# probabilists/zuko

Hardware: AMD Instinct MI355X
Metric: log_prob samples/sec, NSF d=64 K=8 bins=8 batch=2^20 (higher is better)
Workload: dtype f32; 1 GPU; NSF(features=64, context=0, transforms=8, bins=8, hidden=[256]*3) log_prob, batch=2^20 per GPU, x~N(0,1), seed-0 init; batch_per_gpu=1048576, global_batch=1048576, parallelism=batch-sharded x1, one RCCL all-reduce of the scalar NLL

## Files before the change

include/zuko_amd.h:

```cpp
#ifndef ZUKO_AMD_H
#define ZUKO_AMD_H

#include <stdint.h>

#ifdef __cplusplus
extern "C" {
#endif

#define ZK_DTYPE_F32 0
#define ZK_DTYPE_F64 1
#define ZK_DTYPE_BF16 2

#define ZK_ACT_NONE 0
#define ZK_ACT_RELU 1
#define ZK_ACT_ELU 2
#define ZK_ACT_TANH 3
#define ZK_ACT_SILU 4
#define ZK_ACT_GELU 5
#define ZK_ACT_SIGMOID 6
#define ZK_ACT_LEAKY 7


int zk_rqs_forward(int dtype, int64_t N, int64_t D, int K, double bound, double slope, const void* x,
                   const void* widths, int64_t w_sN, int64_t w_sD, const void* heights, int64_t h_sN, int64_t h_sD,
                   const void* derivs, int64_t d_sN, int64_t d_sD, void* y, void* ladj, int ladj_reduced,
                   int32_t* bin_out, void* stream);

int zk_rqs_inverse(int dtype, int64_t N, int64_t D, int K, double bound, double slope, const void* y,
                   const void* widths, int64_t w_sN, int64_t w_sD, const void* heights, int64_t h_sN, int64_t h_sD,
                   const void* derivs, int64_t d_sN, int64_t d_sD, void* x, int32_t* bin_out, void* stream);

int zk_rqs_from_knots(int dtype, int inverse, int64_t N, int64_t D, int K, const void* in, const void* horizontal,
                      const void* vertical, const void* slopes, int64_t k_sN, int64_t k_sD, void* out, void* ladj,
                      int32_t* bin_out, void* stream);

int zk_rqs_diag(int inverse, int64_t N, int64_t D, int K, double bound, double slope, const void* in, const void* widths,
                int64_t w_sN, int64_t w_sD, const void* heights, int64_t h_sN, int64_t h_sD, const void* derivs, int64_t d_sN,
                int64_t d_sD, void* out, void* ladj, int32_t* bin_out, float* knots_out, void* stream);

int zk_affine_forward(int dtype, int64_t N, int64_t D, double slope, const void* x, const void* shift, int64_t s_sN,
                      int64_t s_sD, const void* scale, int64_t c_sN, int64_t c_sD, void* y, void* ladj, int ladj_reduced,
                      void* stream);
int zk_affine_inverse(int dtype, int64_t N, int64_t D, double slope, const void* y, const void* shift, int64_t s_sN,
                      int64_t s_sD, const void* scale, int64_t c_sN, int64_t c_sD, void* x, void* stream);

int zk_sos_forward(int dtype, int64_t N, int64_t D, int P, int L1, double slope, const double* gl_nodes01,
                   const double* gl_weights01, const void* x, const void* a_coef, int64_t a_sN, int64_t a_sD,
                   const void* constant, int64_t c_sN, int64_t c_sD, void* y, void* ladj, int ladj_reduced, void* stream);
int zk_sos_inverse(int dtype, int64_t N, int64_t D, int P, int L1, double slope, const double* gl_nodes01,
                   const double* gl_weights01, int n_bisect, const void* y, const void* a_coef, int64_t a_sN,
                   int64_t a_sD, const void* constant, int64_t c_sN, int64_t c_sD, void* x, void* stream);

int zk_bernstein_forward(int dtype, int64_t N, int64_t D, int M, int bounded, double bound, double eps, const void* x,
                         const void* theta, int64_t t_sN, int64_t t_sD, void* y, void* ladj, int ladj_reduced, void* stream);
int zk_bernstein_inverse(int dtype, int64_t N, int64_t D, int M, int bounded, double bound, double eps, int n_bisect, const void* y,
                         const void* theta, int64_t t_sN, int64_t t_sD, void* x, void* stream);

int zk_gauss_forward(int dtype, int64_t N, int64_t D, int K, const void* x, const void* shift, int64_t b_sN, int64_t b_sD,
                     const void* scale, int64_t a_sN, int64_t a_sD, void* y, void* ladj, int ladj_reduced, void* stream);
int zk_gauss_inverse(int dtype, int64_t N, int64_t D, int K, double bound, int n_bisect, const void* y, const void* shift,
                     int64_t b_sN, int64_t b_sD, const void* scale, int64_t a_sN, int64_t a_sD, void* x, void* stream);

int zk_linear(int dtype, int64_t N, int in_features, int out_features, const void* x, int64_t ldx, const void* weight,
              const uint8_t* mask, const void* bias, int act, void* y, int64_t ldy, void* stream);

int zk_linear_bf16(int64_t N, int in_features, int out_features, const void* x, int64_t ldx, const void* weight, const uint64_t* tile_live_mask,
                   const void* bias, int act, void* y, int64_t ldy, void* stream);

int zk_linear_bf16_rqs(int64_t N, int in_features, int panels, const void* h, int64_t ldh, const void* weight_panels, const uint64_t* tile_live_mask,
                       const void* bias_panels, int K, int features, double bound, double slope, const void* x, int64_t ldx, void* y, int64_t ldy,
                       float* partial, float* ladj, void* stream);
int zk_linear_bf16_rqs_lanes(int64_t N, int in_features, int panels, const void* h, int64_t ldh, const void* weight_panels,
                             const uint64_t* tile_live_mask, const void* bias_panels, int K, int features, double bound, double slope, const void* x,
                             int64_t ldx, void* y, int64_t ldy, float* partial, float* ladj, void* stream);

typedef struct zk_ar_args_v1 {
  uint32_t struct_size;
  uint32_t version;
  int32_t uni_kind;
  int32_t D;
  int32_t DIN;
  int32_t n_layers;
  int32_t n_groups;
  int32_t n_chunks;
  int32_t act;
  int32_t bias_floats;
  int32_t accumulate;
  int32_t rev;
  int32_t n_sched;
  int32_t g0;
  int32_t g1;
  int32_t reserved;
  int64_t N;
  int64_t ldx;
  int64_t ldy;
  int64_t ldo;
  int64_t ldphi;
  double bound;
  double slope;
  const void* x;
  void* y;
  void* ladj;
  const void* y_in;
  void* x_out;
  const void* wstream;
  const void* bias;
  const uint32_t* skip;
  const int32_t* featmap;
  int32_t* bin_out;
  float* knots_out;
  const int32_t* sched;
  const int32_t* olim;
  const void* launcher;
  void* h1;
  void* h2;
  void* h3;
  void* phi;
  void* gh1;
  void* gh2;
  void* gh3;
  int32_t phi_packed;
  int32_t pad_;
  const double* gl_nodes01;
  const double* gl_weights01;
  double eps;
  double wdescale0;
  double wdescale1;
  double wdescale2;
  double wdescale3;
  uint32_t* amax0;
  uint32_t* amax1;
  uint32_t* amax2;
  uint32_t* amax3;
  const void* base_loc;
  const void* base_scale;
} zk_ar_args_v1;

int zk_ar_forward(const zk_ar_args_v1* args, void* stream);
int zk_ar_forward_split(const zk_ar_args_v1* args, void* stream);
int zk_ar_forward_diag(const zk_ar_args_v1* args, void* stream);
int zk_ar_dgrad_chain(const zk_ar_args_v1* args, void* stream);
int zk_ar_dgrad_full(const zk_ar_args_v1* args, void* stream);
int zk_ar_backward_full(const zk_ar_args_v1* args, void* stream);
int zk_ar_inverse_sweep(const zk_ar_args_v1* args, void* stream);
int zk_ar_inverse_partial(const zk_ar_args_v1* args, void* stream);
typedef struct zk_coupling_args_v1 {
  uint32_t struct_size;
  uint32_t version;
  int32_t D;
  int32_t C;
  int32_t nit;
  int32_t n_groups;
  int32_t n_layers;
  int32_t n_chunks;
  int32_t act;
  int32_t bias_floats;
  int32_t accumulate;
  int32_t static_ok;
  int64_t N;
  int64_t ldx;
  int64_t ldc;
  int64_t ldy;
  double slope;
  const void* in;
  const void* ctx;
  void* out;
  void* ladj;
  const void* wstream;
  const void* bias;
  const int32_t* bias_off;
  const int32_t* amap;
  const int32_t* fmap;
  const int32_t* tiles;
  const int32_t* widths;
  double wdescale0;
  double wdescale1;
  double wdescale2;
  double wdescale3;
} zk_coupling_args_v1;
int zk_coupling_forward(const zk_coupling_args_v1* args, void* stream);
int zk_coupling_inverse(const zk_coupling_args_v1* args, void* stream);
typedef struct zk_ar_inc_args_v1 {
  uint32_t struct_size;
  uint32_t version;
  int32_t uni_kind;
  int32_t n_hidden;
  int32_t D;
  int32_t C;
  int32_t n_groups;
  int32_t n_chunks;
  int32_t act;
  int32_t bias_floats;
  int64_t N;
  int64_t ldy;
  int64_t ldc;
  int64_t ldx;
  double bound;
  double slope;
  const void* y;
  const void* ctx;
  void* x;
  void* ladj;
  const void* wstream;
  const void* bias;
  const int32_t* bias_off;
  const int32_t* featmap;
  const int32_t* prog;
  int32_t half;
  int32_t pad_;
  double wdescale1;
  double wdescale2;
  double wdescale3;
  const double* gl_nodes01;
  const double* gl_weights01;
  double eps;
  int32_t n_bisect;
  int32_t pad2_;
} zk_ar_inc_args_v1;
int zk_ar_inverse_incremental(const zk_ar_inc_args_v1* args, void* stream);
int zk_ar_inc_lds_bytes(int bias_floats, int nit);
int zk_ar_lds_bytes(int variant, int bias_floats);
int zk_ar_forward_static(const zk_ar_args_v1* args, void* stream);
int zk_ar_forward_train(const zk_ar_args_v1* args, void* stream);
int zk_gather_f32(const void* src, const uint8_t* mask, const int32_t* idx, int64_t n, void* dst, void* stream);
int zk_gather_split_bf16(const void* src, const uint8_t* mask, const int32_t* idx, int64_t n_blocks, void* dst, void* stream);
int zk_gather_split_f16(const void* src, const uint8_t* mask, const int32_t* idx, int64_t n_blocks, void* dst, double scale, void* stream);
typedef struct zk_gather_desc_v1 {
  uint32_t struct_size;
  int32_t split;
  int64_t count;
  const void* src;
  const uint8_t* mask;
  const int32_t* idx;
  void* dst;
} zk_gather_desc_v1;
int zk_gather_multi(int n, const zk_gather_desc_v1* descs, void* stream);

int zk_univariate_backward(int kind, int64_t N, int64_t D, int K, double bound, double slope, const void* x, const void* phi,
                           const void* gy, const void* gl, int gl_reduced, void* gx, void* gphi, void* stream);
int zk_sos_backward(int64_t N, int64_t D, int P, int L1, double slope, const double* gl_nodes01, const double* gl_weights01,
                    int has_const, const void* x, const void* params, const void* gy, const void* gl, int gl_reduced, void* gx,
                    void* gparams, void* stream);
int zk_bernstein_backward(int64_t N, int64_t D, int M, int bounded, double bound, double eps, const void* x, const void* theta, const void* gy,
                          const void* gl, int gl_reduced, void* gx, void* gtheta, void* stream);
int zk_gauss_backward(int64_t N, int64_t D, int K, const void* x, const void* phi, const void* gy, const void* gl, int gl_reduced,
                      void* gx, void* gphi, void* stream);
int zk_inverse_seed(int64_t n, const void* gx, const void* ladj, void* gy, void* seed, void* stream);
int zk_diag_normal_backward(int64_t N, int64_t D, const void* z, const void* loc, const void* scale, const void* g, void* gz,
                            void* stream);
int zk_act_backward(int64_t n, const void* y, const void* gout, int act, void* gin, void* stream);

int zk_gemm_f32_skip(int64_t N, int in_features, int out_features, const void* x, int64_t ldx, const void* w, const uint64_t* kskip,
                     const void* bias, int act, const void* gate, int64_t ldg, int gate_act, void* y, int64_t ldy, void* stream);
int zk_wgrad_slices(int64_t N, int npairs);
int zk_wgrad_f32(int64_t N, int out_features, int in_features, const void* g, int64_t ldg, const void* h, int64_t ldh,
                 const int32_t* pairs, int npairs, float* partial, const uint8_t* mask, void* dw, int accumulate, const int32_t* rows,
                 const int32_t* cols, void* stream);
int zk_wgrad_bias_f32(int64_t N, int out_features, int in_features, const void* g, int64_t ldg, const void* h, int64_t ldh,
                      const int32_t* pairs, int npairs, float* partial, const uint8_t* mask, void* dw, int accumulate,
                      const uint8_t* cs_flag, float* cs_partial, void* db, const int32_t* rows, const int32_t* cols, void* stream);
typedef struct zk_wgrad_layer_v1 {
  uint32_t struct_size;
  int32_t out_features;
  int32_t in_features;
  int32_t npairs;
  int64_t ldg;
  int64_t ldh;
  const void* g;
  const void* h;
  const int32_t* pairs;
  void* partial;
  const uint8_t* mask;
  void* dw;
  const uint8_t* cs_flag;
  void* cs_partial;
  void* db;
  const int32_t* rows;
  const int32_t* cols;
  const uint32_t* g_amax;
  const uint32_t* h_amax;
} zk_wgrad_layer_v1;
int zk_wgrad_multi(int n_layers, const zk_wgrad_layer_v1* layers, int64_t N, void* stream);
int zk_colsum_slices(int64_t N);
int zk_colsum_f32(int64_t N, int C, const void* x, int64_t ld, float* workspace, void* out, int accumulate, void* stream);

#define ZK_AMAX_WORDS 2048
typedef struct zk_amax_desc_v1 {
  uint32_t struct_size;
// ... 282 lines not shown
```

zuko_amd/csrc/fused_ar.hip:

```cpp
#include "../../include/zuko_amd.h"
#include "zk_ar_common.h"
#include <type_traits>

#ifndef ZK_AR_TIMING
#define ZK_AR_TIMING 0
#endif

namespace zk {

template <int CH, int NR> struct RingT {
  static constexpr int kChunk = CH, kSlots = NR;
  float* lds;
  const float* stream;
  int n_chunks, pos, slot, load_chunk, load_slot, wave, lane, dbg;
  const int* sched;

  template <int I> __device__ __forceinline__ void dma(const float* g, float* l) {
    if constexpr (I < CH / AR_WAVES) {
#ifndef ZK_AR_NO_RING_DMA
      __builtin_amdgcn_global_load_lds((const __attribute__((address_space(1))) void*)g, (__attribute__((address_space(3))) void*)l, 16, I * AR_TF * 4, 0);
#endif
      dma<I + 1>(g, l);
    }
  }
// ... 336 lines not shown

int zk_gather_multi(int n, const zk_gather_desc_v1* descs, void* stream) {
  if (n < 1 || n > 8 || !descs) return ZK_EINVAL;
  GatherMulti m{};
  m.n = n;
  int blocks = 0;
  for (int k = 0; k < n; ++k) {
    const zk_gather_desc_v1& d = descs[k];
    if (d.struct_size != sizeof(zk_gather_desc_v1) || d.count < 0 || (d.count > 0 && (!d.src || !d.idx || !d.dst))) return ZK_EINVAL;
    if (d.split && (((uintptr_t)d.idx % 16) || ((uintptr_t)d.dst % 16))) return ZK_EINVAL;
    m.g[k] = {(const float*)d.src, d.mask, d.idx, d.count, d.dst, d.split};
    m.start[k] = blocks;
    const int64_t threads = d.split ? d.count * 64 : d.count;
    if (threads > (int64_t)0x7fffffff) return ZK_EINVAL;
    blocks += (int)((threads + 255) / 256);
  }
  m.start[n] = blocks;
  if (blocks == 0) return 0;
  hipLaunchKernelGGL(gather_multi_kernel, dim3((unsigned)blocks), dim3(256), 0, (hipStream_t)stream, m);
  return ZK_LAUNCH_CHECK();
}

#ifndef AR_CH
#define AR_CH 24
#define AR_NR 3
#endif
typedef RingT<AR_CH, AR_NR> Ring24x3;
static int ar_lds_bytes(int bias_floats, bool xlds, int xs) { return ArLds::bytes(AR_CH * AR_NR * AR_TF, bias_floats, xlds ? AR_WAVES : 0, xs); }
int zk_ar_lds_bytes(int variant, int bias_floats) { return ar_lds_bytes(bias_floats, true, 260); }

struct ArPartial {
  const void* static_fn = nullptr;
  int rev = 0;
  float* act_out[3] = {nullptr, nullptr, nullptr};
  float* phi_out = nullptr;
  int64_t ldphi = 0;
  int phi_packed = 0;
  const double* gl_nodes01 = nullptr;
  const double* gl_weights01 = nullptr;
  double eps = 0.0;
  int32_t* bin_out = nullptr;
  float* knots_out = nullptr;
  double wdescale[4] = {0.0, 0.0, 0.0, 0.0};
  unsigned* amax[4] = {nullptr, nullptr, nullptr, nullptr};
  const float* base_loc = nullptr;
  const float* base_scale = nullptr;
  const int* sched = nullptr;
  int n_sched = 0;
  const int* olim = nullptr;
  int g0 = 0, g1 = -1;
};

static int ar_launch(const ArPartial& part, bool inverse, int uni_kind, int64_t N, int D, int DIN, const void* x, int64_t ldx, const void* yin, int64_t ldyin, void* y, int64_t ldy,
                     void* ladj, int accumulate, const void* wstream, const void* bias, int bias_floats, const uint32_t* skip, const int32_t* featmap,
                     int n_layers, int n_groups, int n_chunks, int act, double bound, double slope, int variant, void* stream) {
  if (N <= 0) return 0;
  if (n_groups * 8 > ArLds::FMAP_WORDS || n_groups > ArLds::SKIP_WORDS) return ZK_EINVAL;
  if (n_layers < 2 || DIN > (part.static_fn ? 512 : 256) || DIN < D || DIN % 4 || ldx % 4 || ((uintptr_t)x % 16) || n_chunks < 1) return ZK_EINVAL;
  ArArgs a{};
  a.N = N; a.D = D; a.DIN = DIN;
  a.x = (const float*)x; a.ldx = ldx;
  a.yin = (const float*)yin; a.ldyin = ldyin;
  a.y = (float*)y; a.ldy = ldy; a.ladj = (float*)ladj; a.accumulate = accumulate;
  a.stream = (const float*)wstream; a.bias = (const float*)bias; a.skip = skip; a.featmap = featmap;
  a.L = n_layers; a.NG = n_groups; a.n_chunks = n_chunks; a.act = act; a.bias_floats = bias_floats;
  a.bound = (float)bound; a.ls = (float)log(slope);
  a.lc = rqs_lean_const(bound, log(slope));
  a.n_tiles = (N + 127) / 128;
  a.g0 = 0; a.g1 = n_groups;
  for (int l = 0; l < 8; ++l) a.olim[l] = 3;
  if (part.sched) {
    if (part.n_sched < 1 || part.g0 < 0 || part.g1 > n_groups || part.g0 >= part.g1 || n_layers - 1 > 8) return ZK_EINVAL;
    a.sched = part.sched; a.n_sched = part.n_sched; a.g0 = part.g0; a.g1 = part.g1;
    for (int l = 0; l < n_layers - 1; ++l) a.olim[l] = part.olim[l];
  }
#if ZK_AR_TIMING
  a.dbg = (variant >> 8) & 0xff;
  if ((variant & 0xff) != 0) return ZK_EINVAL;
#else
  if (variant != 0) return ZK_EINVAL;
#endif
  if (part.static_fn) {
    if (inverse || part.sched || ((part.bin_out != nullptr) != (part.knots_out != nullptr))) return ZK_EINVAL;
    a.bin_out = part.bin_out; a.knots_out = part.knots_out;
    a.l1rev = part.rev;
    for (int l = 0; l < 3; ++l) a.act_out[l] = part.act_out[l];
    a.phi_out = part.phi_out; a.ldphi = part.ldphi; a.phi_packed = part.phi_packed;
    if (uni_kind == 5) {
      const bool conditioner_only = part.phi_out != nullptr && y == nullptr;
      if ((!part.gl_nodes01 || !part.gl_weights01) && !conditioner_only) return ZK_EINVAL;
      a.sos.bound = (float)bound; a.sos.slope = (float)slope; a.sos.P = 3; a.sos.L1 = 5;
      if (part.gl_nodes01 && part.gl_weights01)
        for (int i = 0; i < 5; ++i) { a.sos.node[i] = (float)part.gl_nodes01[i]; a.sos.weight[i] = (float)part.gl_weights01[i]; }
    }
    a.eps = (float)(part.eps > 0.0 ? part.eps : 1e-6);
    for (int l = 0; l < 4; ++l) a.wdescale[l] = (float)part.wdescale[l];
    for (int l = 0; l < 4; ++l) a.amax[l] = part.amax[l];
    if ((part.base_loc != nullptr) != (part.base_scale != nullptr) || (part.base_loc && (!ladj || part.phi_out || part.bin_out))) return ZK_EINVAL;
    a.base_loc = part.base_loc; a.base_scale = part.base_scale;
    return ((ars_launch_fn)part.static_fn)(&a, ARS_ABI, (int)sizeof(ArArgs), part.phi_out != nullptr, stream);
  }
  a.xs = ((D + 3) / 4) * 4 + 4;
  const bool vec_ok = (D % 4 == 0) && (ldy % 4 == 0) && ((uintptr_t)y % 16 == 0) && (!inverse || ((ldyin % 4 == 0) && ((uintptr_t)yin % 16 == 0)));
  a.xlds = vec_ok && ar_lds_bytes(bias_floats, true, a.xs) <= 160 * 1024;
  const int lds = ar_lds_bytes(bias_floats, a.xlds, a.xs);
  if (lds > 160 * 1024) return ZK_EINVAL;
  const void* fn = nullptr;
#define ZK_AR_PICK(UNI)                                                                                                                     \
  (inverse ? (a.xlds ? (const void*)ar_kernel<UNI, true, Ring24x3, true> : (const void*)ar_kernel<UNI, true, Ring24x3, false>)            \
           : (a.xlds ? (const void*)ar_kernel<UNI, false, Ring24x3, true> : (const void*)ar_kernel<UNI, false, Ring24x3, false>))
#define ZK_AR_PICK_X(UNI) (inverse ? (const void*)ar_kernel<UNI, true, Ring24x3, true> : (const void*)ar_kernel<UNI, false, Ring24x3, true>)
  if (uni_kind == 0) fn = ZK_AR_PICK(UniAffine);
  else if (uni_kind == 1) fn = ZK_AR_PICK(UniRqs8);
  else if (uni_kind >= 2 && uni_kind <= 4 && !a.xlds) return ZK_EINVAL;
  else if (uni_kind == 2) fn = ZK_AR_PICK_X(UniRqs4);
  else if (uni_kind == 3) fn = ZK_AR_PICK_X(UniRqs16);
  else if (uni_kind == 4) fn = ZK_AR_PICK_X(UniCircRqs8);
  else return ZK_EINVAL;
  if (part.bin_out || part.knots_out) {
    if (inverse || part.sched || !a.xlds || !part.bin_out || !part.knots_out) return ZK_EINVAL;
    a.bin_out = part.bin_out; a.knots_out = part.knots_out;
    if (uni_kind == 1) fn = (const void*)ar_kernel<UniRqs8, false, Ring24x3, true, true>;
    else if (uni_kind == 2) fn = (const void*)ar_kernel<UniRqs4, false, Ring24x3, true, true>;
    else if (uni_kind == 3) fn = (const void*)ar_kernel<UniRqs16, false, Ring24x3, true, true>;
    else return ZK_EINVAL;
  }
  return ar_launch_dyn_lds(fn, 256, 512, lds, a, stream);
}

#define AR_ARGS_OK(args) (ar_args_norm(args, &args##_norm_) ? ((args) = &args##_norm_, true) : false)

static int ar_launch_v1(const ArPartial& part, bool inverse, const zk_ar_args_v1& p, void* stream) {
  return ar_launch(part, inverse, p.uni_kind, p.N, p.D, p.DIN, p.x, p.ldx, inverse ? p.y_in : nullptr, inverse ? p.ldy : 0, inverse ? p.x_out : p.y, inverse ? p.ldo : p.ldy,
                   inverse ? nullptr : p.ladj, p.accumulate, p.wstream, p.bias, p.bias_floats, p.skip, p.featmap, p.n_layers, p.n_groups, p.n_chunks, p.act, p.bound, p.slope, 0,
                   stream);
}

int zk_ar_forward(const zk_ar_args_v1* args, void* stream) {
  zk_ar_args_v1 args_norm_;
  if (!AR_ARGS_OK(args)) return ZK_EINVAL;
  return ar_launch_v1(ArPartial{}, false, *args, stream);
}

int zk_ar_forward_diag(const zk_ar_args_v1* args, void* stream) {
  zk_ar_args_v1 args_norm_;
  if (!AR_ARGS_OK(args)) return ZK_EINVAL;
  ArPartial part;
  part.bin_out = args->bin_out; part.knots_out = args->knots_out;
  zk_ar_args_v1 p = *args;
  p.accumulate = 0;
  return ar_launch_v1(part, false, p, stream);
}

int zk_ar_forward_static(const zk_ar_args_v1* args, void* stream) {
  zk_ar_args_v1 args_norm_;
  if (!AR_ARGS_OK(args) || !args->launcher) return ZK_EINVAL;
  ArPartial part;
  part.static_fn = args->launcher; part.rev = args->rev;
  part.gl_nodes01 = args->gl_nodes01; part.gl_weights01 = args->gl_weights01; part.eps = args->eps;
  part.bin_out = args->bin_out; part.knots_out = args->knots_out;
  part.wdescale[0] = args->wdescale0; part.wdescale[1] = args->wdescale1; part.wdescale[2] = args->wdescale2; part.wdescale[3] = args->wdescale3;
  part.base_loc = (const float*)args->base_loc; part.base_scale = (const float*)args->base_scale;
  zk_ar_args_v1 p = *args;
  p.skip = nullptr;
  return ar_launch_v1(part, false, p, stream);
}

int zk_ar_forward_train(const zk_ar_args_v1* args, void* stream) {
  zk_ar_args_v1 args_norm_;
  if (!AR_ARGS_OK(args) || !args->launcher || !args->phi || !args->h1) return ZK_EINVAL;
  const int n_layers = args->n_layers;
  if (n_layers < 2 || n_layers > 4 || (n_layers > 2 && !args->h2) || (n_layers > 3 && !args->h3)) return ZK_EINVAL;
  if (((uintptr_t)args->h1 % 16) || ((uintptr_t)args->h2 % 16) || ((uintptr_t)args->h3 % 16)) return ZK_EINVAL;
  ArPartial part;
  part.static_fn = args->launcher; part.rev = args->rev;
  part.act_out[0] = (float*)args->h1; part.act_out[1] = (float*)args->h2; part.act_out[2] = (float*)args->h3; part.phi_out = (float*)args->phi; part.ldphi = args->ldphi;
  part.phi_packed = args->phi_packed;
  part.amax[0] = args->amax0; part.amax[1] = args->amax1; part.amax[2] = args->amax2; part.amax[3] = args->amax3;
  zk_ar_args_v1 p = *args;
  p.act = 1; p.skip = nullptr;
  if (!p.y) {
    p.ldy = 0; p.ladj = nullptr; p.accumulate = 0; p.bound = 1.0; p.slope = 1e-3;
  }
  return ar_launch_v1(part, false, p, stream);
}

typedef int (*ars_dgrad_fn)(const ArArgs* a, int abi, int args_bytes, void* stream);
static bool ar_chain_args_ok(const zk_ar_args_v1* args) {
  return args->launcher && args->x && args->y && args->wstream && args->n_layers >= 2 && args->n_layers <= 4 && args->N >= 0 && args->N <= 0x7fffffff;
}
static ArArgs ar_chain_args(const zk_ar_args_v1* args, int chain_layers, int gated) {
  const void* hs[3] = {args->h1, args->h2, args->h3};
  void* gs[3] = {args->gh1, args->gh2, args->gh3};
  ArArgs a{};
  a.x = (const float*)args->x; a.ldx = args->ldx; a.N = args->N; a.D = args->D; a.DIN = args->DIN; a.L = chain_layers; a.n_chunks = args->n_chunks;
  a.stream = (const float*)args->wstream;
  a.phi_out = (float*)args->y; a.ldphi = args->ldy;
  for (int c = 0; c < gated; ++c) {
    a.gate[c] = (const float*)hs[gated - 1 - c];
    a.act_out[c] = (float*)gs[gated - 1 - c];
  }
  return a;
}
static int ar_chain_launch(const zk_ar_args_v1* args, const ArArgs& a, void* stream) { return ((ars_dgrad_fn)args->launcher)(&a, ARS_ABI, (int)sizeof(ArArgs), stream); }

int zk_ar_dgrad_chain(const zk_ar_args_v1* args, void* stream) {
  zk_ar_args_v1 args_norm_;
  if (!AR_ARGS_OK(args) || !ar_chain_args_ok(args)) return ZK_EINVAL;
  if (args->N == 0) return 0;
  return ar_chain_launch(args, ar_chain_args(args, args->n_layers - 1, args->n_layers - 2), stream);
}

int zk_ar_dgrad_full(const zk_ar_args_v1* args, void* stream) {
  zk_ar_args_v1 args_norm_;
  if (!AR_ARGS_OK(args) || !ar_chain_args_ok(args)) return ZK_EINVAL;
  if (args->N == 0) return 0;
  ArArgs a = ar_chain_args(args, args->n_layers, args->n_layers - 1);
  a.accumulate = args->accumulate;
  return ar_chain_launch(args, a, stream);
}

int zk_ar_backward_full(const zk_ar_args_v1* args, void* stream) {
  zk_ar_args_v1 args_norm_;
  if (!AR_ARGS_OK(args) || !ar_chain_args_ok(args) || !args->phi || !args->x_out || !args->y_in || !args->ladj || !args->featmap) return ZK_EINVAL;
  if (args->uni_kind < 0 || args->uni_kind > 1 || args->DIN < args->D || args->D < 1) return ZK_EINVAL;
  if (args->N == 0) return 0;
  ArArgs a = ar_chain_args(args, args->n_layers, args->n_layers - 1);
  a.NG = args->n_groups; a.featmap = args->featmap; a.accumulate = args->accumulate;
  a.gy = (const float*)args->y_in; a.ldgy = args->ldo; a.gl = (const float*)args->ladj;
  a.phi_in = (const float*)args->phi; a.gphi_out = (float*)args->x_out; a.ldpin = args->ldphi; a.phi_packed = 1;
  a.bound = (float)args->bound; a.ls = (float)log(args->slope);
  a.amax[0] = args->amax0; a.amax[1] = args->amax1; a.amax[2] = args->amax2; a.amax[3] = args->amax3;
  return ar_chain_launch(args, a, stream);
}

int zk_ar_inverse_sweep(const zk_ar_args_v1* args, void* stream) {
  zk_ar_args_v1 args_norm_;
  if (!AR_ARGS_OK(args)) return ZK_EINVAL;
  return ar_launch_v1(ArPartial{}, true, *args, stream);
}

int zk_ar_inverse_partial(const zk_ar_args_v1* args, void* stream) {
  zk_ar_args_v1 args_norm_;
  if (!AR_ARGS_OK(args) || !args->sched || !args->olim) return ZK_EINVAL;
  ArPartial part;
  part.sched = args->sched; part.n_sched = args->n_sched; part.olim = args->olim; part.g0 = args->g0; part.g1 = args->g1;
  return ar_launch_v1(part, true, *args, stream);
}

}
```

zuko_amd/csrc/fused_ar_half_impl.h:

```cpp
#pragma once
#include "fused_ar_split_impl.h"

#ifndef ARH_LOOK
#define ARH_LOOK 1
#endif
#ifndef ARH_RELU_INT
#define ARH_RELU_INT 0
#endif
#ifndef ARH_EPI_PINNED
#define ARH_EPI_PINNED 1
#endif
#ifndef ARH_DESCALE_PK
#define ARH_DESCALE_PK 1
#endif
#ifndef ARH_PREFETCH
#define ARH_PREFETCH 1
#endif

namespace zk {

typedef _Float16 f16x8 __attribute__((ext_vector_type(8)));

struct ArhB {
  f16x8 h, l;
};

__device__ __forceinline__ void arh_scale(float& amax, float& s, float& inv_s) {
  amax = fmaxf(amax, __shfl_xor(amax, 16, 64));
  amax = fmaxf(amax, __shfl_xor(amax, 32, 64));
  int e = __builtin_amdgcn_frexp_expf(amax);
  int ea = 15 - e;
  ea = ea > 90 ? 90 : (ea < -90 ? -90 : ea);
  s = __builtin_amdgcn_ldexpf(1.0f, ea);
  inv_s = __builtin_amdgcn_ldexpf(1.0f, -ea);
}

#define ARH_AMAX_OVERFLOW (65520.f * 0x1p90f)

typedef unsigned arh_u32x4 __attribute__((ext_vector_type(4)));
typedef float arh_f32x2 __attribute__((ext_vector_type(2)));

__device__ __forceinline__ void arh_split(const f32x4& lo, const f32x4& hi, float s, ArhB& b) {
  if (ARX_ABL == 6) {
    b.h = __builtin_bit_cast(f16x8, lo); b.l = __builtin_bit_cast(f16x8, hi);
    return;
  }
#if ARH_EPI_PINNED
  const float nz = -0.f;
  arh_u32x4 h, l;
#pragma unroll
  for (int e = 0; e < 4; ++e) asm("v_fma_mixlo_f16 %0, %1, %2, %3" : "=v"(h[e]) : "v"(e < 2 ? lo[2 * e] : hi[2 * e - 4]), "v"(s), "s"(nz));
#pragma unroll
  for (int e = 0; e < 4; ++e) asm("v_fma_mixhi_f16 %0, %1, %2, %3" : "+v"(h[e]) : "v"(e < 2 ? lo[2 * e + 1] : hi[2 * e - 3]), "v"(s), "s"(nz));
#pragma unroll
  for (int e = 0; e < 4; ++e) asm("v_fma_mixlo_f16 %0, %1, %2, -%3 op_sel:[0,0,0] op_sel_hi:[0,0,1]" : "=v"(l[e]) : "v"(e < 2 ? lo[2 * e] : hi[2 * e - 4]), "v"(s), "v"(h[e]));
#pragma unroll
  for (int e = 0; e < 4; ++e) asm("v_fma_mixhi_f16 %0, %1, %2, -%3 op_sel:[0,0,1] op_sel_hi:[0,0,1]" : "+v"(l[e]) : "v"(e < 2 ? lo[2 * e + 1] : hi[2 * e - 3]), "v"(s), "v"(h[e]));
  b.h = __builtin_bit_cast(f16x8, h); b.l = __builtin_bit_cast(f16x8, l);
  return;
#endif
#pragma unroll
  for (int e = 0; e < 8; ++e) {
    const float v = (e < 4 ? lo[e] : hi[e - 4]) * s;
    const _Float16 h = (_Float16)v;
    const float r = v - (float)h;
    b.h[e] = h;
    b.l[e] = (_Float16)r;
  }
}

#define ARH_MFMA(A, B, C) C = __builtin_amdgcn_mfma_f32_16x16x32_f16(__builtin_bit_cast(f16x8, A), B, C, 0, 0, 0)
__device__ __forceinline__ void arh_block(const f32x4 (&a)[2], const ArhB& b, f32x4& c) {
  if (ARX_ABL == 2) {
    asm volatile("" ::"v"(a[0]), "v"(a[1]));
    return;
  }
  ARH_MFMA(a[1], b.h, c);
  ARH_MFMA(a[0], b.l, c);
  ARH_MFMA(a[0], b.h, c);
}

__device__ __forceinline__ void arh_touch(f32x4& v) { asm volatile("" : "+v"(v)); }
template <int N> __device__ __forceinline__ void arh_settle(f32x4& a0, f32x4& a1) { asm volatile("s_waitcnt lgkmcnt(%2)" : "+v"(a0), "+v"(a1) : "n"(N)); }
template <int N> __device__ __forceinline__ void arh_settle(f32x4& a0, f32x4& a1, f32x4& a2) { asm volatile("s_waitcnt lgkmcnt(%3)" : "+v"(a0), "+v"(a1), "+v"(a2) : "n"(N)); }

template <int WAVES, int CH, int NR> struct ArhRing : ArRingS<WAVES, CH, NR> {
  typedef ArRingS<WAVES, CH, NR> B;
  template <int XV> __device__ __forceinline__ void advance_x() {
    asm volatile("s_waitcnt vmcnt(%0) lgkmcnt(0)" ::"n"((NR - 2) * B::PER + XV) : "memory");
    if (ARX_ABL != 4) __builtin_amdgcn_s_barrier();
    asm volatile("" ::: "memory");
    this->issue();
    this->slot = (this->slot + 1 == NR) ? 0 : this->slot + 1;
    this->cur_off = this->lds_off + (unsigned)(this->slot * CH * AR_TF * 4 + this->lane * 16);
  }
  template <int S, int XV = 0> __device__ __forceinline__ f32x4 read() {
    if constexpr (XV != 0 && S % CH == 0) {
      advance_x<XV>();
      f32x4 v;
      if (ARX_ABL == 5) {
        asm volatile("v_mov_b32 %0, %1" : "=v"(v[0]) : "v"(this->cur_off));
        v[1] = v[2] = v[3] = v[0];
        return v;
      }
      asm volatile("ds_read_b128 %0, %1 offset:%2" : "=v"(v) : "v"(this->cur_off), "n"((S % CH) * AR_TF * 4));
      return v;
    } else {
      return B::template read<S>();
    }
  }
};

template <int WAVES, int CH, int IMAGES, int BPOS> struct ArhRing4 {
  static constexpr int NR = 4, PER = CH / WAVES, PIVOT = PER > 4 ? 4 : 0, CHB = CH * AR_TF * 4, NCH = (IMAGES + CH - 1) / CH;
  static_assert(PER * WAVES == CH && PER <= 6 && BPOS % 2 == 0 && BPOS >= 2 * (ARH_LOOK + 1) && BPOS + 1 < CH && CH % 2 == 0 && IMAGES % 2 == 0, "ring geometry");
  static constexpr int trigger(int c) {
    const int last = (IMAGES < (c + 1) * CH ? IMAGES : (c + 1) * CH) - 1;
    return c * CH + BPOS + 1 < last ? c * CH + BPOS + 1 : last;
  }
  static constexpr int first_trigger_from(int pos) {
    for (int c = 0; c < NCH; ++c)
      if (trigger(c) >= pos) return trigger(c);
    return -1;
  }
  const char* gsrc;
  char* ldst;
  unsigned goff, gend;
  unsigned fill_off;
  unsigned read_off;
  unsigned lane_off;
  unsigned lane16;
  unsigned cur_off;
  __device__ __forceinline__ void start(float* lds, const float* stream, int n_chunks, int wave, int lane) {
    const int b0 = wave * PER + PIVOT;
    gsrc = reinterpret_cast<const char*>(stream + b0 * AR_TF);
    ldst = reinterpret_cast<char*>(lds + b0 * AR_TF);
    goff = 0; gend = (unsigned)n_chunks * CHB; fill_off = 0;
    lane16 = (unsigned)lane * 16;
    lane_off = (unsigned)(size_t)((__attribute__((address_space(3))) float*)lds) + lane16;
#pragma unroll
    for (int i = 0; i < NR - 1; ++i) issue();
    read_off = (NR - 1) * CHB;
    cur_off = lane_off;
  }
  template <int I> __device__ __forceinline__ void dma(const char* g, char* l) {
    if constexpr (I < PER) {
      __builtin_amdgcn_global_load_lds((const __attribute__((address_space(1))) void*)g, (__attribute__((address_space(3))) void*)l, 16, (I - PIVOT) * AR_TF * 4, 0);
      dma<I + 1>(g, l);
    }
  }
  __device__ __forceinline__ void issue() {
    asm volatile("" : "+v"(lane16));
    if (ARX_ABL != 1) dma<0>(gsrc + goff + (size_t)lane16, ldst + fill_off);
    goff = (goff + CHB == gend) ? 0 : goff + CHB;
    fill_off = (fill_off + CHB == NR * CHB) ? 0 : fill_off + CHB;
  }
  template <int XV, bool DRAIN> __device__ __forceinline__ void boundary() {
    if constexpr (DRAIN) asm volatile("s_waitcnt vmcnt(%0) lgkmcnt(0)" ::"n"(XV) : "memory");
    else asm volatile("s_waitcnt vmcnt(%0)" ::"n"(XV) : "memory");
    if (ARX_ABL != 4) __builtin_amdgcn_s_barrier();
    asm volatile("" ::: "memory");
    issue();
    asm volatile("" ::: "memory");
  }
  template <int S, int XV = 0> __device__ __forceinline__ f32x4 read() {
    static_assert(S >= 0 && S < IMAGES, "stream position");
    if constexpr (S % CH == 0) {
      read_off = (read_off + CHB == NR * CHB) ? 0 : read_off + CHB;
      cur_off = lane_off + read_off;
    }
    f32x4 v;
    if (ARX_ABL == 5) {
      asm volatile("v_mov_b32 %0, %1" : "=v"(v[0]) : "v"(cur_off));
      v[1] = v[2] = v[3] = v[0];
    } else {
      asm volatile("ds_read_b128 %0, %1 offset:%2" : "=v"(v) : "v"(cur_off), "n"((S % CH) * AR_TF * 4));
    }
    if constexpr (S == trigger(S / CH)) boundary<XV, (S % CH != BPOS + 1)>();
    return v;
  }
};

template <class S, int L, class Ring> __device__ __forceinline__ void arh_hidden(Ring& ring, const float* bias_q, const ArhB (&in)[S::TMAX / 2], f32x4 (&out)[S::TMAX], float d) {
  typedef ArxPat<S> P;
  constexpr int NB = S::NB[L], BASE = S::BASE[L], HTL = S::HT[L];
  ars_for<HTL>([&](auto t_) ARS_ALWAYS_INLINE {
    constexpr int t = t_;
    if constexpr (!P::tile_has_blocks(L, t)) out[t] = *reinterpret_cast<const f32x4*>(bias_q + t * 16);
  });
  if constexpr (NB > 0) {
    constexpr int LOOK = ARH_LOOK < NB ? ARH_LOOK : NB;
    f32x4 a[LOOK + 1][2];
    f32x4 bs;
    f32x4 acc;
    const unsigned bias_addr = arx_lds_addr(bias_q);
    ars_for<LOOK>([&](auto b_) ARS_ALWAYS_INLINE {
      constexpr int b = b_;
      ars_for<2>([&](auto p) ARS_ALWAYS_INLINE { a[b][p] = ring.template read<BASE + 2 * b + decltype(p)::value>(); });
    });
    ars_for<NB>([&](auto s_) ARS_ALWAYS_INLINE {
      constexpr int s = s_, ot = P::ot(L, s), ip = P::ip(L, s), cur = s % (LOOK + 1);
      constexpr bool first_of_tile = (s == 0 || P::ot(L, s - 1) != ot), last_of_tile = (s + 1 == NB || P::ot(L, s + 1) != ot);
      if constexpr (first_of_tile) acc = f32x4{0.f, 0.f, 0.f, 0.f};
      if constexpr (last_of_tile) bs = arx_lds_raw<ot * 64>(bias_addr);
      if constexpr (s + LOOK < NB) {
        constexpr int nx = (s + LOOK) % (LOOK + 1);
        ars_for<2>([&](auto p) ARS_ALWAYS_INLINE { a[nx][p] = ring.template read<BASE + 2 * (s + LOOK) + decltype(p)::value>(); });
      }
      constexpr int ahead = (s + LOOK < NB ? LOOK : NB - 1 - s);
      if constexpr (last_of_tile) arh_settle<(s + LOOK < NB ? 2 : 0)>(a[cur][0], a[cur][1], bs);
      else arh_settle<2 * ahead>(a[cur][0], a[cur][1]);
      if (ARX_FENCE) __builtin_amdgcn_sched_barrier(0);
      arh_block(a[cur], in[ip], acc);
      if (ARX_FENCE) __builtin_amdgcn_sched_barrier(0);
      if constexpr (last_of_tile) {
        if (ARH_DESCALE_PK) {
#pragma unroll
          for (int r = 0; r < 4; r += 2) {
            const arh_f32x2 o = __builtin_elementwise_fma(arh_f32x2{acc[r], acc[r + 1]}, arh_f32x2{d, d}, arh_f32x2{bs[r], bs[r + 1]});
            out[ot][r] = o[0]; out[ot][r + 1] = o[1];
          }
        } else {
#pragma unroll
          for (int r = 0; r < 4; ++r) out[ot][r] = __builtin_fmaf(acc[r], d, bs[r]);
        }
      }
    });
  }
}

template <class S, int L, class Ring> __device__ __forceinline__ void arh_hidden_stack(Ring& ring, const float* bias_lds, int q, ArhB (&in)[S::TMAX / 2], f32x4 (&out)[S::TMAX], const ArArgs& a,
                                                                                       float& inv_s, float& poison) {
  if constexpr (L < S::NH) {
    arh_hidden<S, L>(ring, bias_lds + L * S::BIAS_STRIDE + 4 * q, in, out, a.wdescale[L] * inv_s);
    constexpr int HTL = S::HT[L];
    float amax = 0.f;
    if constexpr (S::ACT == 1 && ARH_EPI_PINNED) {
#pragma unroll
      for (int t = 0; t < HTL; ++t)
#pragma unroll
        for (int r = 0; r < 4; r += 2) {
          asm("v_max_f32 %0, 0, %0" : "+v"(out[t][r]));
          asm("v_max_f32 %0, 0, %0" : "+v"(out[t][r + 1]));
          asm("v_max3_f32 %0, %0, %1, %2" : "+v"(amax) : "v"(out[t][r]), "v"(out[t][r + 1]));
        }
    } else if constexpr (S::ACT == 1) {
#pragma unroll
      for (int t = 0; t < HTL; ++t)
#pragma unroll
        for (int r = 0; r < 4; ++r) {
          if (ARH_RELU_INT) out[t][r] = __builtin_bit_cast(float, max(__builtin_bit_cast(int, out[t][r]), 0));
          else out[t][r] = out[t][r] < 0.f ? 0.f : out[t][r];
          amax = fmaxf(amax, out[t][r]);
        }
    } else {
      ar_activate<S::ACT, HTL>(out, out);
#pragma unroll
      for (int t = 0; t < HTL; ++t)
#pragma unroll
        for (int r = 0; r < 4; ++r) amax = fmaxf(amax, fabsf(out[t][r]));
    }
    float s;
    arh_scale(amax, s, inv_s);
    if constexpr (S::ACT == 1 && ARH_EPI_PINNED) {
      if (!(amax < ARH_AMAX_OVERFLOW)) poison = __builtin_nanf("");
    }
    const f32x4 zero = {0.f, 0.f, 0.f, 0.f};
#pragma unroll
    for (int p = 0; p < (HTL + 1) / 2; ++p) arh_split(out[2 * p], 2 * p + 1 < HTL ? out[2 * p + 1] : zero, s, in[p]);
    arh_hidden_stack<S, L + 1, Ring>(ring, bias_lds, q, in, out, a, inv_s, poison);
  }
}

template <class S, typename Uni, bool DIAG, bool TERM> __device__ __forceinline__ void arh_body(const ArArgs& a) {
  constexpr bool RING4 = S::NR == 4;
  typedef std::conditional_t<RING4, ArhRing4<S::WAVES, S::CH, S::IMAGES, S::BPOS>, ArhRing<S::WAVES, S::CH, S::NR>> Ring;
  static_assert(S::WAVES == 8 && (S::NR == 3 || S::NR == 4) && S::TMAX <= 16 && S::TMAX % 2 == 0 && S::OCC == 2, "two-part split kernels: widths <= 256, two wavefronts per SIMD");
  constexpr int NT = Uni::NT, FPL = Uni::FPL, TOTAL = Uni::TOTAL, WAVES = S::WAVES;
  constexpr int NG = S::NG;
  constexpr int NSTEP = S::GOFF[NG];
  static_assert(S::IMAGES == S::LAST_BASE + 2 * NSTEP * NT && (S::IMAGES + S::CH - 1) / S::CH == S::NCHUNK, "stream length");
  constexpr bool XLDS = S::XLDS;
  const ArLane ln;
  const int tid = ln.tid, lane = ln.lane, wave = ln.wave, j = ln.j, q = ln.q;

  Ring ring;
  if constexpr (RING4) {
    ring.start(ars_lds, a.stream, a.n_chunks, wave, lane);
  } else {
    ring.lds = ars_lds; ring.stream = a.stream; ring.n_chunks = a.n_chunks; ring.wave = wave; ring.lane = lane;
    ring.load_chunk = 0; ring.load_slot = 0;
#pragma unroll
    for (int i = 0; i < S::NR - 1; ++i) ring.issue();
    ring.slot = S::NR - 1;
    ring.lds_off = (unsigned)(size_t)((__attribute__((address_space(3))) float*)ars_lds);
    ring.cur_off = ring.lds_off;
  }

  auto x_request = [&](int64_t tile, f32x4 (&xv)[S::NIT]) ARS_ALWAYS_INLINE {
    const int64_t n = tile * (16 * WAVES) + wave * 16 + j;
    const float* row = a.x + (n < a.N ? n : a.N - 1) * a.ldx;
#pragma unroll
    for (int it = 0; it < S::NIT; ++it) {
      const int col = it * 16 + 4 * q;
      xv[it] = *reinterpret_cast<const f32x4*>(row + ((it + 1) * 16 <= S::DIN || col < S::DIN ? col : S::DIN - 4));
    }
  };
  f32x4 xnext[S::NIT];
  if (ARH_PREFETCH) x_request(blockIdx.x, xnext);

  float* const bias_lds = ars_lds + S::NR * S::CH * AR_TF;
  int* const fmap_lds = ArLds::fmap(bias_lds, a.bias_floats);
  float* const xr = ArLds::row(fmap_lds, wave, j, a.xs);
  float* const base = ArLds::base(fmap_lds, NG * 4 * FPL);
  if constexpr (TERM) ArLds::stage_base<64 * WAVES>(a, tid, base, S::D);
  ArLds::stage<64 * WAVES>(a, tid, bias_lds, fmap_lds, NG * 4 * FPL);
  const float* bias_last = bias_lds + S::NH * S::BIAS_STRIDE;
  const unsigned bias_last_addr = arx_lds_addr(bias_last + 4 * q);
  const ArFids<NG, FPL, (NG * FPL <= 32)> fids(fmap_lds, q);

  for (int64_t tile = blockIdx.x; tile < a.n_tiles; tile += gridDim.x) {
    const int64_t n = tile * (16 * WAVES) + wave * 16 + j;
    const bool live = n < a.N;
    const int64_t nc = live ? n : a.N - 1;
    const float* xrow = a.x + nc * a.ldx;

    ArhB in[S::TMAX / 2];
    f32x4 out[S::TMAX];
    float poison;
    float inv_s;
    {
      f32x4 xin[S::NIT + 1];
#pragma unroll
      for (int it = 0; it < S::NIT; ++it) {
        f32x4 v = {0.f, 0.f, 0.f, 0.f};
        if (ARH_PREFETCH) {
          if ((it + 1) * 16 <= S::DIN || it * 16 + 4 * q < S::DIN) v = xnext[it];
        } else {
          if ((it + 1) * 16 <= S::DIN || it * 16 + 4 * q < S::DIN) v = *reinterpret_cast<const f32x4*>(xrow + it * 16 + 4 * q);
        }
        xin[it] = v;
      }
      xin[S::NIT] = f32x4{0.f, 0.f, 0.f, 0.f};
      poison = ar_poison_of<S::NIT>(xin);
      float amax = 0.f;
#pragma unroll
      for (int it = 0; it < S::NIT; ++it)
#pragma unroll
        for (int r = 0; r < 4; ++r) amax = fmaxf(amax, fabsf(xin[it][r]));
      if constexpr (XLDS) ar_rows_in<S::D>(xr, q, xin);
      float s;
      arh_scale(amax, s, inv_s);
      if constexpr (S::ACT == 1 && ARH_EPI_PINNED) {
        if (!(amax < ARH_AMAX_OVERFLOW)) poison = __builtin_nanf("");
      }
#pragma unroll
      for (int p = 0; p < (S::NIT + 1) / 2; ++p) arh_split(xin[2 * p], xin[2 * p + 1], s, in[p]);
    }

    float ladj_in = 0.f;
    if (ARH_PREFETCH && a.ladj && a.accumulate && live && q == 0) ladj_in = a.ladj[n];

    arh_hidden_stack<S, 0, Ring>(ring, bias_lds, q, in, out, a, inv_s, poison);

    const float dl = a.wdescale[S::NH] * inv_s;
    float lacc = 0.f;
    constexpr int NBL = NSTEP * NT;
    constexpr int LOOKL = ARH_LOOK < NBL ? ARH_LOOK : NBL;
    f32x4 w[LOOKL + 1][2];
    constexpr int XPOS = []() constexpr {
      if constexpr (!ARH_PREFETCH) return -1;
      else if constexpr (RING4) return Ring::first_trigger_from(S::LAST_BASE);
      else return (S::LAST_BASE + S::CH - 1) / S::CH * S::CH;
    }();
    if (ARH_PREFETCH) {
      asm volatile("" ::: "memory");
      x_request(tile + gridDim.x < a.n_tiles ? tile + gridDim.x : tile, xnext);
      asm volatile("" ::: "memory");
    }
#define ARH_READ_LAST(POS) ring.template read<(POS), ((POS) == XPOS ? S::NIT : 0)>()
    ars_for<LOOKL>([&](auto b_) ARS_ALWAYS_INLINE {
      constexpr int b = b_;
      ars_for<2>([&](auto p) ARS_ALWAYS_INLINE { w[b][p] = ARH_READ_LAST(S::LAST_BASE + 2 * b + decltype(p)::value); });
    });
    ars_for<NG>([&](auto g_) ARS_ALWAYS_INLINE {
      constexpr int g = g_, ST0 = S::GOFF[g], GN = S::GOFF[g + 1] - S::GOFF[g];
      int fid[FPL];
      float xin[FPL];
      fids.template fetch<XLDS>(g, xr, xrow, fid, xin);
      float bv[3 * FPL];
      if constexpr (TERM) fids.fetch_base(fid, base, S::D, bv);
      f32x4 acc[NT], bs[NT];
      if constexpr (GN == 0) {
        const float* bg = bias_last + (g * NT) * 16 + 4 * q;
        ars_for<NT>([&](auto t) ARS_ALWAYS_INLINE { bs[t] = *reinterpret_cast<const f32x4*>(bg + t * 16); });
      }
      ars_for<NT>([&](auto t) ARS_ALWAYS_INLINE { acc[t] = f32x4{0.f, 0.f, 0.f, 0.f}; });
      ars_for<GN>([&](auto i_) ARS_ALWAYS_INLINE {
        constexpr int st = ST0 + decltype(i_)::value, ip = S::G_IP[st];
        ars_for<NT>([&](auto t_) ARS_ALWAYS_INLINE {
          constexpr int t = t_, blk = st * NT + t, cur = blk % (LOOKL + 1);
          constexpr bool last_of_group = (decltype(i_)::value == GN - 1 && t == NT - 1);
          if constexpr (last_of_group) {
            ars_for<NT>([&](auto u) ARS_ALWAYS_INLINE { bs[u] = arx_lds_raw<(g * NT + decltype(u)::value) * 64>(bias_last_addr); });
          }
          if constexpr (blk + LOOKL < NBL) {
            constexpr int nx = (blk + LOOKL) % (LOOKL + 1);
            ars_for<2>([&](auto p) ARS_ALWAYS_INLINE { w[nx][p] = ARH_READ_LAST(S::LAST_BASE + 2 * (blk + LOOKL) + decltype(p)::value); });
          }
          constexpr int ahead = (blk + LOOKL < NBL ? LOOKL : NBL - 1 - blk);
          if constexpr (last_of_group) arh_settle<(blk + LOOKL < NBL ? 2 : 0)>(w[cur][0], w[cur][1]);
          else arh_settle<2 * ahead>(w[cur][0], w[cur][1]);
          if constexpr (last_of_group) {
#pragma unroll
            for (int u = 0; u < NT; ++u) arh_touch(bs[u]);
          }
          if (ARX_FENCE) __builtin_amdgcn_sched_barrier(0);
          arh_block(w[cur], in[ip], acc[t]);
          if (ARX_FENCE) __builtin_amdgcn_sched_barrier(0);
        });
      });
      float p[4 * NT];
      ars_for<NT>([&](auto t) ARS_ALWAYS_INLINE {
#pragma unroll
        for (int r = 0; r < 4; ++r) {
          p[4 * t + r] = __builtin_fmaf(acc[t][r], dl, bs[t][r]);
          if (ARH_POISON_ONE) asm("" : "+v"(p[4 * t + r]));
        }
      });
      ar_uni_epilogue<Uni, DIAG, XLDS, true, TERM>(p, a, fid, xin, poison, xr, n, live, S::D, lacc, bv);
    });
#undef ARH_READ_LAST
    if (ARH_PREFETCH) ar_ladj_store<true>(a, lacc, n, live, q, ladj_in);
    if constexpr (XLDS && !TERM) ar_rows_out<S::D>(xr, q, a.y + n * a.ldy, live);
    if (!ARH_PREFETCH) ar_ladj_store(a, lacc, n, live, q);
  }
  asm volatile("s_waitcnt vmcnt(0)" ::: "memory");
}

template <class S, typename Uni, bool DIAG = false> __global__ __launch_bounds__(64 * S::WAVES, S::OCC) void arh_kernel(ArArgs a) { arh_body<S, Uni, DIAG, false>(a); }
template <class S, typename Uni> __global__ __launch_bounds__(64 * S::WAVES, S::OCC) void arht_kernel(ArArgs a) { arh_body<S, Uni, false, true>(a); }

template <class S, typename Uni> static int arh_launch(const ArArgs* in, int abi, int args_bytes, int train, void* stream) {
  if (abi != ARS_ABI || args_bytes != (int)sizeof(ArArgs)) return ZK_EINVAL;
  ArArgs a = *in;
  if (train || a.D != S::D || a.DIN != S::DIN || a.L != S::NH + 1 || a.act != S::ACT || a.sched || a.NG != S::NG || a.n_chunks != S::NCHUNK || a.l1rev) return ZK_EINVAL;
  for (int l = 0; l <= S::NH; ++l)
    if (!(a.wdescale[l] > 0.f) || !(a.wdescale[l] < __builtin_inff())) return ZK_EINVAL;
  a.n_tiles = (a.N + 16 * S::WAVES - 1) / (16 * S::WAVES);
  a.xs = ((S::D + 3) / 4) * 4 + 4;
  const bool term = a.base_loc != nullptr;
  if (term && (!a.base_scale || !a.ladj || a.bin_out || a.knots_out || !ArLds::base_fits(S::NG * 4 * Uni::FPL, S::D))) return ZK_EINVAL;
  const bool vec_ok = (S::D % 4 == 0) && (term || ((a.ldy % 4 == 0) && ((uintptr_t)a.y % 16 == 0)));
  if (S::XLDS != 0 && !vec_ok) return ZK_EINVAL;
  a.xlds = S::XLDS;
  const int lds = ArLds::bytes(S::NR * S::CH * AR_TF, a.bias_floats, S::XLDS ? S::WAVES : 0, a.xs);
  if (lds > 160 * 1024) return ZK_EINVAL;
  const void* fn = nullptr;
  if ((a.bin_out != nullptr) != (a.knots_out != nullptr)) return ZK_EINVAL;
  if (term) {
    fn = (const void*)arht_kernel<S, Uni>;
  } else if (a.bin_out) {
    if constexpr (Uni::NKNOT > 1) fn = (const void*)arh_kernel<S, Uni, true>;
  } else {
    fn = (const void*)arh_kernel<S, Uni, false>;
  }
  if (!fn) return ZK_EINVAL;
  return ar_launch_dyn_lds(fn, 256, 64 * S::WAVES, lds, a, stream);
}

}
```

zuko_amd/csrc/zk_ar_common.h:

```cpp
#pragma once
#include "zk_univariate.h"
#include <cstddef>
#include <cstring>

namespace zk {

typedef float f32x4 __attribute__((ext_vector_type(4)));

#define AR_TF 256
#define AR_WAVES 8
#define AR_T 16
#define ARS_ABI 10
#ifndef ARX_ABL
#define ARX_ABL 0
#endif
#ifndef ARH_POISON_ONE
#define ARH_POISON_ONE 1
#endif

struct ArArgs {
  int64_t N;
  int D, DIN;
  const float* x; int64_t ldx;
  float* y; int64_t ldy;
  const float* yin; int64_t ldyin;
  float* ladj; int accumulate;
  const float* stream;
  const float* bias;
  const uint32_t* skip;
  const int32_t* featmap;
  int L, NG, n_chunks, act, bias_floats, dbg;
  const int* sched;
  int n_sched;
  int olim[8];
  int g0, g1;
  int xlds;
  int xs;
  float bound, ls;
  RqsLeanConst lc;
  int64_t n_tiles;
  int32_t* bin_out;
  float* knots_out;
  int l1rev;
  float* act_out[3];
  float* phi_out;
  int64_t ldphi;
  const float* gate[3];
  const float* phi_in;
  float* gphi_out;
  int64_t ldpin;
  const float* gy; int64_t ldgy;
  const float* gl;
  int phi_packed;
  SosConst<float> sos;
  float eps;
  float wdescale[4];
  unsigned* amax[4];
  const float* base_loc;
  const float* base_scale;
};

__device__ __forceinline__ float act_f32(float v, int act) {
  switch (act) {
    case 1: return v < 0.f ? 0.f : v;
    case 2: return v > 0.f ? v : expm1f(v);
    case 3: return tanhf(v);
    case 4: return v / (1.f + expf(-v));
    case 5: return 0.5f * v * (1.f + erff(v * 0.70710678118654752440f));
    case 6: return 1.f / (1.f + expf(-v));
    case 7: return v > 0.f ? v : 0.01f * v;
    default: return v;
  }
}


struct UniAffine {
  static constexpr int TOTAL = 2, FPL = 2, NT = 1;
  template <bool INV> static __device__ __forceinline__ void poison(float* p, int base, float nan_or_zero) {
    p[base + 0] += nan_or_zero;
    p[base + 1] += nan_or_zero;
  }
  static constexpr int NKNOT = 1;
  template <typename P, typename A> static __device__ __forceinline__ void fwd(const P& p, int base, const A& a, float x, float& y, float& lj, int* k = nullptr, float* ks = nullptr) {
    affine_fwd<float, MathFast>(p(base + 0), p(base + 1), a.ls, x, y, lj);
  }
  template <typename P, typename A> static __device__ __forceinline__ float inv(const P& p, int base, const A& a, float y) {
    return affine_inv<float, MathFast>(p(base + 0), p(base + 1), a.ls, y);
  }
};

template <int K, bool CIRC> struct UniRqs {
  static constexpr int TOTAL = 3 * K - 1, FPL = 1, NT = (TOTAL + 3) / 4;
  static __device__ __forceinline__ float shift(float v, float bound) {
    const float period = 2.f * bound;
    float r = fmodf(v, period);
    r = (r < 0.f) ? r + period : r;
    return r - bound;
  }
  template <bool INV> static __device__ __forceinline__ void poison(float* p, int base, float nan_or_zero) {
#if ARH_POISON_ONE
    p[base + (INV ? K : 0)] += nan_or_zero;
#else
#pragma unroll
    for (int j = 0; j < K; ++j) p[base + (INV ? K : 0) + j] += nan_or_zero;
#endif
  }
  static constexpr int NKNOT = K + 1;
  template <typename P, typename A> static __device__ __forceinline__ void fwd(const P& p, int base, const A& a, float x, float& y, float& lj, int* k = nullptr, float* ks = nullptr) {
    int kk;
    rqs_lean<K, false>([&](int j) { return p(base + j); }, [&](int j) { return p(base + K + j); }, [&](int j) { return p(base + 2 * K + j); }, a.lc,
                       CIRC ? shift(x, a.bound) : x, y, lj, kk, ks);
    if (k) *k = kk;
  }
  template <typename P, typename A> static __device__ __forceinline__ float inv(const P& p, int base, const A& a, float y) {
    float x, lj;
    rqs_lean<K, true>([&](int j) { return p(base + j); }, [&](int j) { return p(base + K + j); }, [&](int j) { return p(base + 2 * K + j); }, a.lc, y, x, lj);
    return CIRC ? shift(x, a.bound) : x;
  }
};
template <int P, int L1> struct UniSos {
  static constexpr int TOTAL = P * L1 + 1, FPL = 1, NT = (TOTAL + 3) / 4, NKNOT = 1;
  template <bool INV> static __device__ __forceinline__ void poison(float* p, int base, float nan_or_zero) {
    p[base] += nan_or_zero;
    p[base + P * L1] += nan_or_zero;
  }
  template <typename Pa, typename A> static __device__ __forceinline__ void fwd(const Pa& p, int base, const A& a, float x, float& y, float& lj, int* k = nullptr, float* ks = nullptr) {
    auto ld = [&](int j) { return p(base + j); };
    y = sos_f<float>(Fixed<P>{}, Fixed<L1>{}, a.sos, ld, x) + p(base + P * L1);
    lj = t_log(sos_g<float>(Fixed<P>{}, Fixed<L1>{}, a.sos, ld, x));
  }
};
template <int NC> struct UniBernBounded {
  static constexpr int TOTAL = NC - 5, FPL = 1, NT = (TOTAL + 3) / 4, NKNOT = 1;
  template <bool INV> static __device__ __forceinline__ void poison(float* p, int base, float nan_or_zero) { p[base] += nan_or_zero; }
  template <typename Pa, typename A> static __device__ __forceinline__ void fwd(const Pa& p, int base, const A& a, float x, float& y, float& lj, int* k = nullptr, float* ks = nullptr) {
    float th[NC];
    bern_theta_bounded<float>(Fixed<NC>{}, [&](int j) { return p(base + j); }, a.bound, th);
    const BernTails<float> t = bern_tails<float>(Fixed<NC>{}, th, true, a.bound, a.eps);
    float d;
    bern_fwd<float>(Fixed<NC>{}, th, t, a.bound, x, y, d, a.eps);
    lj = t_log(d);
  }
};
typedef UniSos<3, 5> UniSos3x5;
typedef UniBernBounded<22> UniBern17;
typedef UniRqs<8, false> UniRqs8;
typedef UniRqs<4, false> UniRqs4;
typedef UniRqs<16, false> UniRqs16;
typedef UniRqs<8, true> UniCircRqs8;


struct ArLds {
  static constexpr int FMAP_WORDS = 1024, SKIP_WORDS = 256;
  static constexpr int bytes(int ring_floats, int bias_floats, int row_waves, int xs) {
    return (ring_floats + bias_floats + FMAP_WORDS + SKIP_WORDS + row_waves * 16 * xs) * (int)sizeof(float);
  }
  static __device__ __forceinline__ int* fmap(float* bias, int bias_floats) { return reinterpret_cast<int*>(bias + bias_floats); }
  static __device__ __forceinline__ int* skip(int* fmap_) { return fmap_ + FMAP_WORDS; }
  static __device__ __forceinline__ float* row(int* fmap_, int wave, int j, int xs) {
    return reinterpret_cast<float*>(fmap_ + FMAP_WORDS + SKIP_WORDS) + wave * 16 * xs + j * xs;
  }
  template <int THREADS> static __device__ __forceinline__ void stage(const ArArgs& a, int tid, float* bias, int* fmap_, int n_fmap, int skip0 = 0, int n_skip = 0) {
    for (int i = tid; i < a.bias_floats; i += THREADS) bias[i] = a.bias[i];
    for (int i = tid; i < n_fmap; i += THREADS) fmap_[i] = a.featmap[i];
    for (int i = tid; i < n_skip; i += THREADS) skip(fmap_)[i] = (int)a.skip[skip0 + i];
    __syncthreads();
  }
  static constexpr bool base_fits(int n_fmap, int D) { return n_fmap + 3 * D <= FMAP_WORDS; }
  static __device__ __forceinline__ float* base(int* fmap_, int n_fmap) { return reinterpret_cast<float*>(fmap_ + n_fmap); }
  template <int THREADS> static __device__ __forceinline__ void stage_base(const ArArgs& a, int tid, float* tab, int D) {
    for (int i = tid; i < D; i += THREADS) {
      const float s = a.base_scale[i];
      tab[i] = a.base_loc[i];
      tab[D + i] = 1.f / (2.f * (s * s));
      tab[2 * D + i] = -t_log(s) - 0.91893853320467274178f;
    }
  }
};

struct ArLane {
  int tid, lane, wave, j, q;
  __device__ __forceinline__ ArLane() : tid(threadIdx.x), lane(tid & 63), wave(__builtin_amdgcn_readfirstlane(tid >> 6)), j(lane & 15), q(lane >> 4) {}
};

template <int NIT, int M> __device__ __forceinline__ float ar_poison_of(const f32x4 (&v)[M]) {
  int bad = 0;
#pragma unroll
  for (int it = 0; it < NIT; ++it)
#pragma unroll
    for (int r = 0; r < 4; ++r) bad |= !(fabsf(v[it][r]) < __builtin_inff());
  bad |= __shfl_xor(bad, 16, 64);
  bad |= __shfl_xor(bad, 32, 64);
  return bad ? __builtin_nanf("") : 0.f;
}

template <int D, int M> __device__ __forceinline__ void ar_rows_in(float* xr, int q, const f32x4 (&v)[M]) {
#pragma unroll
  for (int it = 0; it < (D + 15) / 16; ++it)
    if ((it + 1) * 16 <= D || it * 16 + 4 * q < D) *reinterpret_cast<f32x4*>(xr + it * 16 + 4 * q) = v[it];
  asm volatile("" ::: "memory");
  __builtin_amdgcn_wave_barrier();
}
template <int D> __device__ __forceinline__ void ar_rows_out(const float* xr, int q, float* yrow, bool live) {
  asm volatile("" ::: "memory");
  __builtin_amdgcn_wave_barrier();
  if (live) {
#pragma unroll
    for (int it = 0; it < (D + 15) / 16; ++it)
      if ((it + 1) * 16 <= D || it * 16 + 4 * q < D) *reinterpret_cast<f32x4*>(yrow + it * 16 + 4 * q) = *reinterpret_cast<const f32x4*>(xr + it * 16 + 4 * q);
  }
}
template <int ACT, int N, int M> __device__ __forceinline__ void ar_activate(f32x4 (&dst)[M], const f32x4 (&src)[M]) {
  if constexpr (ACT == 1) {
#pragma unroll
// ... 115 lines not shown
```

zuko_amd/flows/autoregressive.py:

```python

from __future__ import annotations

from functools import partial
import math
import os
from math import ceil, prod
from typing import Callable, Sequence

import torch
from torch import BoolTensor, LongTensor, Size, Tensor
from torch.distributions import Transform

import weakref

import torch.nn as nn

from .. import fused
from ..distributions import DiagNormal
from ..lazy import Flow, LazyTransform, UnconditionalDistribution
from ..nn import MaskedLinear, MaskedMLP, _act_code
from ..transforms import AutoregressiveTransform, DependentTransform, MonotonicAffineTransform, MonotonicRQSTransform
from ..utils import broadcast, unpack
from .elementwise import ElementWiseTransform

# ... 477 lines not shown
                st.run_inverse_sweep(buf, y2)
        return buf[:, :D].reshape(batch + (D,)).contiguous() if buf.shape[1] != D else buf.reshape(batch + (D,))


    def _poly_incremental(self, y: Tensor, want_ladj: bool):
        lazy, c = self.lazy, self.c
        if not (y.is_cuda and y.dtype == torch.float32 and y.dim() >= 1 and _incremental_enabled() and _partial_inverse_enabled()) or want_ladj:
            return None
        if torch.is_grad_enabled() and (y.requires_grad or (c is not None and c.requires_grad) or any(p.requires_grad for p in lazy.hyper.parameters())):
            return None
        lay = lazy._fusable_layout()
        if lay is None or lay[0].kind not in (5, 6) or os.environ.get("ZUKO_AMD_FULL_SWEEPS", "0") == "1":
            return None
        inc_state = lazy.incremental_state(y.device)
        if inc_state is None:
            return None
        D = lazy.features
        if y.shape[-1] != D:
            return None
        if c is not None:
            yb, cb = broadcast(y, c, ignore=1)
        else:
            yb, cb = y, None
        batch = yb.shape[:-1]
        inc_state.refresh([m for m in lazy.hyper if isinstance(m, MaskedLinear)])
        c2 = None if cb is None else cb.reshape(-1, cb.shape[-1]).contiguous()
        x2, _ = inc_state.run(yb.reshape(-1, D).contiguous(), c2, False)
        return x2.reshape(batch + (D,))

    def _ordered_inverse(self, y: Tensor) -> Tensor:
        lazy, c = self.lazy, self.c
        mods = list(lazy.hyper) if isinstance(lazy.hyper, torch.nn.Sequential) else []
        grad = torch.is_grad_enabled() and (y.requires_grad or (c is not None and c.requires_grad) or any(p.requires_grad for p in lazy.hyper.parameters()))
        per_feature = isinstance(lazy.univariate, nn.Module) and getattr(lazy.univariate, "per_feature", False)
        grad = grad or (torch.is_grad_enabled() and isinstance(lazy.univariate, nn.Module) and any(p.requires_grad for p in lazy.univariate.parameters()))
        if lazy.order is None or grad or not mods or type(mods[-1]) is not MaskedLinear or not y.is_cuda or y.dtype not in (torch.float32, torch.float64) or os.environ.get("ZUKO_AMD_FULL_SWEEPS", "0") == "1":
            return super()._inverse(y)
        from .. import ops

        if c is not None:
            yb, cb = broadcast(y, c, ignore=1)
        else:
            yb, cb = y, None
        batch = yb.shape[:-1]
        y2 = yb.reshape(-1, lazy.features)
        c2 = None if cb is None else cb.reshape(-1, cb.shape[-1])

        def linear(h, w, b, m, act_module):
            code = None if act_module is None else _act_code(act_module)
            if act_module is None or code is not None:
                return ops.linear(h, w, b, m, code or 0)
            return act_module(ops.linear(h, w, b, m))

        if per_feature:
            x2 = wavefront_inverse(lazy, y2, c2, self.passes, linear, lambda phi, ys, idx: lazy.univariate(*unpack(phi, lazy.shapes), features=idx).inv(ys), with_features=True)
        else:
            x2 = wavefront_inverse(lazy, y2, c2, self.passes, linear, lambda phi, ys: lazy.univariate(*unpack(phi, lazy.shapes)).inv(ys))
        return x2.reshape(batch + (lazy.features,))


def wavefront_inverse(lazy: "MaskedAutoregressiveTransform", y2: Tensor, c2: Tensor | None, passes: int, linear, inverse_of, stack=None, with_features: bool = False) -> Tensor:
    from ..nn import apply_stack

    stack = apply_stack if stack is None else stack

    mods = list(lazy.hyper)
    D, total, last = lazy.features, lazy.total, mods[-1]
    dev = y2.device
    x2 = torch.zeros_like(y2)
    units = lazy._sweep_units(dev, passes)
    if units is not None:
        hbuf = [y2.new_zeros((y2.shape[0], m.weight.shape[0])) for m in mods[0:-1:2]]
        urows = lazy._sweep_unit_rows(dev, passes) if y2.dtype == mods[0].weight.dtype else None
    sweep_no = {}
    for s_, idx in lazy._sweep_features(dev, passes):
        if units is None:
            h = stack(mods[:-1], x2 if c2 is None else torch.cat((x2, c2), dim=-1))
        else:
            h = x2 if c2 is None else torch.cat((x2, c2), dim=-1)
            for l, lin in enumerate(mods[0:-1:2]):
                first_t = sweep_no.get(l, 0)
                todo = [units[l][t] for t in range(first_t, s_ + 1) if units[l][t] is not None]
                sweep_no[l] = s_ + 1
                if todo:
                    u_ = todo[0] if len(todo) == 1 else torch.cat(todo)
                    if urows is not None:
                        wr, mr, br, starts = urows[l]
                        r0, r1 = starts[first_t], starts[s_ + 1]
                        w_, m_, bias = wr[r0:r1], mr[r0:r1], None if br is None else br[r0:r1]
                    else:
                        w_, m_, bias = lin.weight.index_select(0, u_), lin.mask.index_select(0, u_), None if lin.bias is None else lin.bias.index_select(0, u_)
                    hbuf[l].index_copy_(1, u_, linear(h, w_, bias, m_, mods[2 * l + 1]))
                h = hbuf[l]
        if isinstance(idx, tuple):
            lo, hi = idx
            rows, k = slice(lo * total, hi * total), hi - lo
            w, b, m, ys = last.weight[rows], None if last.bias is None else last.bias[rows], last.mask[rows], y2[:, lo:hi]
        else:
            rows, k = (idx[:, None] * total + torch.arange(total, device=dev)[None, :]).reshape(-1), idx.numel()
            w, b, m, ys = last.weight.index_select(0, rows), None if last.bias is None else last.bias.index_select(0, rows), last.mask.index_select(0, rows), y2.index_select(1, idx)
        phi = linear(h, w, b, m, None).unflatten(-1, (k, total))
        xs = inverse_of(phi, ys, idx) if with_features else inverse_of(phi, ys)
        if isinstance(idx, tuple):
            x2[:, idx[0] : idx[1]] = xs
        else:
            x2[:, idx] = xs
    return x2


class _FusedInverse(Transform):

    domain = AutoregressiveTransform.codomain
    codomain = AutoregressiveTransform.domain
    bijective = True

    def __init__(self, fwd: FusedAutoregressiveTransform) -> None:
        super().__init__()
        self._fwd = fwd

    @property
    def inv(self) -> Transform:
        return self._fwd

    def _call(self, y: Tensor) -> Tensor:
        return self._fwd._inverse(y)

    def _inverse(self, x: Tensor) -> Tensor:
        return self._fwd._call(x)

    def log_abs_det_jacobian(self, y: Tensor, x: Tensor) -> Tensor:
        return -self._fwd.log_abs_det_jacobian(x, y)

    def call_and_ladj(self, y: Tensor):
        x, ladj = self._fwd.inverse_and_ladj(y)
        return x, -ladj


class MAF(Flow):

    def __init__(self, features: int, context: int = 0, transforms: int = 3, randperm: bool = False, **kwargs) -> None:
        ascending = torch.arange(features)
        fixed = [ascending, torch.flipud(ascending)]
        layers = [
            MaskedAutoregressiveTransform(
                features=features,
                context=context,
                order=torch.randperm(features) if randperm else fixed[i % 2],
                **kwargs,
            )
            for i in range(transforms)
        ]
        base = UnconditionalDistribution(DiagNormal, loc=torch.zeros(features), scale=torch.ones(features), buffer=True)
        super().__init__(layers, base)
```

zuko_amd/fused.py:

```python

from __future__ import annotations

from dataclasses import dataclass

import ctypes
import math
import os

import numpy as np
import torch
from torch import Tensor

TILE = 16
CHUNK = 24
GROUP_HIDDEN = 4
MAX_WIDTH = 256
MAX_WIDTH_WIDE = 512


@dataclass
class UniLayout:

    kind: int
    total: int
# ... 251 lines not shown

def partial_schedule(plan: ArPlan, g_lo: int, g_hi: int):
    L = plan.n_layers
    need = 0
    for g in range(g_lo, g_hi):
        need |= int(plan.skip[(L - 1) * 4 + g])
    olim = [0] * (L - 1)
    for l in range(L - 2, -1, -1):
        otgs = sorted({it // GROUP_HIDDEN for it in range(16) if need >> it & 1})
        olim[l] = max(otgs) if otgs else -1
        nxt = 0
        for otg in range(olim[l] + 1):
            nxt |= int(plan.skip[l * 4 + otg])
        need = nxt
    sched = []
    for l in range(L - 1):
        nblk = plan.otg_blocks_end[l][olim[l]] if olim[l] >= 0 else 0
        c0 = plan.layer_block0[l] // plan.chunk
        sched += list(range(c0, c0 + -(-nblk // plan.chunk)))
    for g in range(g_lo, g_hi):
        sched += list(range(plan.group_chunk0[g], plan.group_chunk0[g] + plan.group_nchunks[g]))
    return sched, olim




GS_BLOCKS_PER_CHUNK = 8


def gsplit_gather(plan: ArPlan):
    if plan.max_width > MAX_WIDTH or plan.layout.kind > 4 or plan.group_chunk0:
        return None
    L, n_otg, n_it = plan.n_layers, MAX_WIDTH // TILE // GROUP_HIDDEN, MAX_WIDTH // TILE
    zero = -np.ones((64, 4), dtype=np.int64)

    def finish(blocks):
        pad = -len(blocks) % GS_BLOCKS_PER_CHUNK
        blocks = blocks + [-np.ones((64, 8), dtype=np.int64)] * pad
        return np.stack(blocks).astype(np.int32).reshape(-1) if blocks else np.zeros(0, np.int32)

    gathers = []
    for l in range(L - 1):
        tiles = plan.gather[l].reshape(-1, 64, 4)
        at, k = {}, 0
        for otg in range(n_otg):
            bits = int(plan.skip[l * n_otg + otg])
            for it in range(n_it):
                if bits >> it & 1:
                    for t in range(GROUP_HIDDEN):
                        at[(otg * GROUP_HIDDEN + t, it)] = k
                        k += 1
        blocks = []
        for otg in range(n_otg):
            bits = int(plan.skip[l * n_otg + otg])
            for ip in range(n_it // 2):
                if bits >> (2 * ip) & 3:
                    for t in range(GROUP_HIDDEN):
                        t0, t1 = at.get((otg * GROUP_HIDDEN + t, 2 * ip)), at.get((otg * GROUP_HIDDEN + t, 2 * ip + 1))
                        blocks.append(np.concatenate([zero if t0 is None else tiles[t0], zero if t1 is None else tiles[t1]], axis=1))
        gathers.append(finish(blocks))
    nt = plan.layout.nt
    tiles = plan.gather[L - 1].reshape(-1, 64, 4)
    blocks, k = [], 0
    for g in range(plan.n_groups):
        bits = int(plan.skip[(L - 1) * n_otg + g])
        at = {}
        for it in range(n_it):
            if bits >> it & 1:
                at[it] = k
                k += nt
        for ip in range(n_it // 2):
            if bits >> (2 * ip) & 3:
                for t in range(nt):
                    t0, t1 = at.get(2 * ip), at.get(2 * ip + 1)
                    blocks.append(np.concatenate([zero if t0 is None else tiles[t0 + t], zero if t1 is None else tiles[t1 + t]], axis=1))
    gathers.append(finish(blocks))
    offsets, cursor = [], 0
    for g in gathers:
        offsets.append(cursor * 768)
        cursor += len(g) // 512
    return gathers, offsets, max(1, cursor // GS_BLOCKS_PER_CHUNK)



_PRECISIONS = {"f16x2": "f16x2", "high": "f16x2", "bf16x3": "bf16x3", "highest": "bf16x3"}
_precision = None


def matmul_precision() -> str:
    global _precision
    if _precision is None:
        _precision = _PRECISIONS.get(os.environ.get("ZUKO_AMD_MATMUL", "f16x2").lower(), "f16x2")
    return _precision


def set_matmul_precision(mode: str) -> None:
    global _precision
    if mode.lower() not in _PRECISIONS:
        raise ValueError(f"zuko_amd.set_matmul_precision: unknown mode '{mode}' (one of {sorted(_PRECISIONS)})")
    _precision = _PRECISIONS[mode.lower()]


HALF_SPREAD_LOG2 = 14
HALF_SMALL_FRACTION = 0.01
HALF_ROW_LOG2 = 12
HALF_MIN_LOG2, HALF_MAX_LOG2 = -20, 40


def half_scales(linears):
    stats = []
    for m in linears:
        w = m.weight.detach()
        a = (w * m.mask).abs() if getattr(m, "mask", None) is not None else w.abs()
        big = a.amax()
        nz = a > 0
        small = (nz & (a < big * 2.0 ** -HALF_SPREAD_LOG2)).sum() / nz.sum().clamp_min(1)
        rowmax = a.amax(dim=1)
        minrow = torch.where(rowmax > 0, rowmax, big).amin()
        bias = getattr(m, "bias", None)
        bfin = torch.isfinite(bias.detach()).all() if bias is not None else torch.ones((), dtype=torch.bool, device=w.device)
        stats.append(torch.stack([big.float(), small.float(), minrow.float(), bfin.float()]))
    out = []
    for big, small, minrow, bfin in torch.stack(stats).tolist():
        if big == 0.0:
            out.append((bfin == 1.0, 0))
            continue
        ok = bfin == 1.0 and math.isfinite(big) and 2.0 ** HALF_MIN_LOG2 <= big <= 2.0 ** HALF_MAX_LOG2 and small <= HALF_SMALL_FRACTION and minrow >= big * 2.0 ** -HALF_ROW_LOG2
        out.append((bool(ok), 15 - math.frexp(big)[1] if math.isfinite(big) else 0))
    return out


@dataclass
class WeightStream:

    gather: list
    offsets: list
    n_chunks: int
    buf: Tensor
    mode: int
    stamp: object = None


def chunk_of(variant: int = 0) -> int:
    return CHUNK


def default_variant() -> int:
    return 0


HALF, GSPLIT, STATIC, GENERIC = range(4)


class FusedAR:

    def __init__(self, plan: ArPlan, device: torch.device, act: int, bound: float, slope: float, variant: int = 0) -> None:
        self.plan = plan
        self.variant = variant
        self.device = device
        self.act = act
        self.bound = bound
        self.slope = slope
        self.skip = torch.from_numpy(plan.skip.view(np.int32).copy()).to(device)
        self.featmap = torch.from_numpy(plan.featmap.copy()).to(device)
        self.gather = [torch.from_numpy(g).to(device) for g in plan.gather]
        self.bias_gather = [torch.from_numpy(g).to(device) for g in plan.bias_gather]
        self.stream = torch.empty(plan.n_blocks * 256, dtype=torch.float32, device=device)
        self.bias_floats = plan.bias_off[-1] + len(plan.bias_gather[-1])
        self.bias = torch.empty(self.bias_floats, dtype=torch.float32, device=device)
        self._stamp = None
        self.generic_ok = plan.max_width <= MAX_WIDTH and plan.layout.kind <= 4
        self.eps = 1e-6
        self._gl = None
        self.static = None
        self._static_tried_rows = self._half_tried_rows = -1
        self.fine = None
        self.half = None
        self.half_stream = None
        self.half_ok = False
        self.half_descale = None
        self._acquire_static(None)
        self.gs_mode = os.environ.get("ZUKO_AMD_GSPLIT", "1")
        self.gs = None
        self._seen_stamp = None

    @property
    def static_variant(self) -> int:
        return 0 if self.static is None else 1 + self.static[1]

    @property
    def _gs_stamp(self):
        return self.gs.stamp if self.gs else None

    def _acquire_static(self, rows) -> None:
        from . import static_ar

        upgradable = self.static is not None and not self.static[0].meta.get("split") and static_ar.split_enabled() and rows is not None
        self._acquire_half(rows)
        if (self.static is not None and not upgradable) or self.plan.fine_gather is None or (rows is not None and rows <= self._static_tried_rows):
            return
        if rows is not None:
            self._static_tried_rows = rows if rows < static_ar.jit_min_rows() else 1 << 62
        found = static_ar.lookup(self.plan, self.plan.layout.kind, self.act, rows)
        if found is not None and (self.static is None or found[0] is not self.static[0]):
            self.static = found
            if found[0].meta.get("split"):
                self.fine = self._table_stream(static_ar.split_tables(self.plan, self.plan.layout.kind, self.act), 1)
            else:
                p = self.plan
                self.fine = self._weight_stream(p.fine_gather, [b * 256 for b in p.fine_layer_block0], p.fine_n_chunks, p.fine_n_chunks * 24 * 256, 0)

    def _weight_stream(self, gathers, offsets, n_chunks: int, floats: int, mode: int) -> WeightStream:
        return WeightStream([torch.from_numpy(g).to(self.device) for g in gathers], offsets, n_chunks, torch.zeros(floats, dtype=torch.float32, device=self.device), mode)

    def _table_stream(self, tg, mode: int) -> WeightStream:
        t, gathers = tg
        return self._weight_stream(gathers, [b * 256 for b in t["BASE"]] + [t["LAST_BASE"] * 256], t["NCHUNK"], t["STREAM_IMAGES"] * 256, mode)

    def _acquire_half(self, rows) -> None:
        from . import static_ar

        if self.half is not None or self.plan.fine_gather is None or not static_ar.half_enabled() or (rows is not None and rows <= self._half_tried_rows):
            return
        if rows is not None:
            self._half_tried_rows = rows if rows < static_ar.jit_min_rows() else 1 << 62
        kern = static_ar.lookup_half(self.plan, self.plan.layout.kind, self.act, rows)
        if kern is not None:
            self.half = kern
            self.half_stream = self._table_stream(static_ar.half_tables(self.plan, self.plan.layout.kind, self.act), 2)

    def _refresh_half(self, linears, stamp) -> None:
        from . import _C
        from .ops import _ptr, _stream

        scales = half_scales(linears)
        ws = self.half_stream
        ws.stamp = stamp
        self.half_ok = all(ok for ok, _ in scales)
        if not self.half_ok:
            return
        self.half_descale = [2.0 ** -e for _, e in scales]
        for l, (m, (_, e)) in enumerate(zip(linears, scales)):
            w = m.weight.detach()
            if not w.is_contiguous():
                w = w.contiguous()
            nb = ws.gather[l].numel() // 512
            if nb:
                _C.check(_C.lib().zk_gather_split_f16(_ptr(w), _ptr(m.mask.contiguous().view(torch.uint8)), _ptr(ws.gather[l]), nb, _ptr(ws.buf[ws.offsets[l] :]), 2.0 ** e, _stream()),
                         "zk_gather_split_f16")

    def static_args(self, launcher, rev: int, ws: WeightStream, **io):
        from . import _C
        from .ops import _ptr

        p = self.plan
        fields = dict(launcher=launcher, rev=rev, uni_kind=p.layout.kind, D=p.features, wstream=_ptr(ws.buf), bias=_ptr(self.bias), bias_floats=self.bias_floats, featmap=_ptr(self.featmap),
                      n_layers=p.n_layers, n_groups=p.n_groups, n_chunks=ws.n_chunks, act=self.act, bound=self.bound, slope=self.slope)
        fields.update(io)
        return _C.args("zk_ar_args_v1", **fields)

    def _half_args(self, **io):
        d = list(self.half_descale) + [1.0] * (4 - len(self.half_descale))
        return self.static_args(self.half.launcher, 0, self.half_stream, wdescale0=d[0], wdescale1=d[1], wdescale2=d[2], wdescale3=d[3], **io)

    def _half_serves(self, y: Tensor | None) -> bool:
        return (self.half is not None and self.half_ok and self.half_stream.stamp is not None and self.half_stream.stamp == self._seen_stamp and matmul_precision() == "f16x2"
                and self.gs_mode != "force" and (y is None or not self.half.meta["XLDS"] or (y.stride(0) % 4 == 0 and y.data_ptr() % 16 == 0)))

    def serves_terminal(self) -> bool:
        p = self.plan
        if p.n_groups * 4 * p.layout.fpl + 3 * p.features > 1024:
            return False
        which = self._product(None)
        return which == HALF or (which == STATIC and bool(self.static[0].meta.get("split")) and p.layout.kind not in (5, 6))

    def _product(self, y: Tensor | None) -> int:
        p = self.plan
        if self._half_serves(y):
            return HALF
        aligned = y is None or (y.stride(0) % 4 == 0 and y.data_ptr() % 16 == 0)
        gs = self._gsplit()
        if gs is not None and gs.stamp is not None and gs.stamp == self._seen_stamp:
            if p.layout.kind <= 1 or (p.features % 4 == 0 and aligned):
                return GSPLIT
            if y is None:
                return GENERIC
        if self.static is not None and (not self.static[0].meta["XLDS"] or aligned):
            return STATIC
        return GENERIC

    def ready(self, rows: int) -> bool:
        from . import static_ar

        self._acquire_static(static_ar.effective_rows(self, rows))
        return self.generic_ok or self.static is not None

    def _gsplit(self):
        from . import static_ar

        if self.gs_mode == "0" or (self.static is not None and self.gs_mode != "force") or not self.generic_ok or not static_ar.split_enabled():
            return None
        if self.gs is None:
            t = gsplit_gather(self.plan)
            if t is None:
                self.gs = False
            else:
# ... 152 lines not shown
```

zuko_amd/static_ar.py:

```python

from __future__ import annotations

import ctypes
import dataclasses
import fcntl
import hashlib
import json
import math
import os
import shutil
import subprocess
import sys
import threading

import numpy as np

HERE = os.path.dirname(os.path.abspath(__file__))
CSRC = os.path.join(HERE, "csrc")
ARS_DIR = os.path.join(HERE, "lib", "ars")
ARS_ABI = 10
UNI_TYPES = {0: "zk::UniAffine", 1: "zk::UniRqs8", 2: "zk::UniRqs4", 3: "zk::UniRqs16", 4: "zk::UniCircRqs8", 5: "zk::UniSos3x5", 6: "zk::UniBern17"}
SPLIT_ONLY_KINDS = {3, 5, 6}
_HEADERS = ("fused_ar_static_impl.h", "fused_ar_split_impl.h", "zk_ar_common.h", "zk_univariate.h", "zk_univariate_bwd.h", "zk_common.h", "zk_half.h")

# ... 149 lines not shown
                    S_IT.append(it)
                    S_MASK.append(m)
                    n += 1
        NS.append(n)
    G_IT, GOFF = [], [0]
    for g in range(plan.n_groups):
        bits = int(plan.skip[NH * n_otg + g])
        G_IT += [it for it in range(32) if bits >> it & 1]
        GOFF.append(len(G_IT))
    waves = 8 if TMAX <= 16 else 4
    D = plan.features
    xs = ((D + 3) // 4) * 4 + 4
    bias_floats = plan.bias_off[-1] + len(plan.bias_gather[-1])
    base = (3 * 24 * 256 + bias_floats + 1024 + 256) * 4
    xlds = int(D % 4 == 0 and base + waves * 16 * xs * 4 <= 160 * 1024)
    if base + (waves * 16 * xs * 4 if xlds else 0) > 160 * 1024:
        return None
    if plan.n_groups * plan.layout.fpl * 4 > 1024:
        return None
    return {
        "uni": int(uni_kind), "ACT": int(act), "D": int(D), "DIN": int(din4), "NIT": int(NIT), "NH": int(NH), "HT": HT, "TMAX": int(TMAX), "NG": int(plan.n_groups),
        "NCHUNK": int(plan.fine_n_chunks), "BIAS_STRIDE": int(plan.max_width), "NS": NS, "S_OTG": S_OTG, "S_IT": S_IT, "S_MASK": S_MASK,
        "BASE": [int(b) for b in plan.fine_layer_block0[:NH]], "LAST_BASE": int(plan.fine_layer_block0[NH]), "GOFF": GOFF, "G_IT": G_IT,
        "WAVES": waves, "XLDS": xlds, "TRAIN_OK": int(act == 1 and NH <= 3 and waves == 8 and all(w % 16 == 0 for w in widths) and uni_kind != 3),
    }


def split_enabled() -> bool:
    return os.environ.get("ZUKO_AMD_EXACT_F32", "0") != "1"


def split_geometry() -> tuple:
    g = os.environ.get("ZUKO_AMD_SPLIT_GEOM", "8x24")
    try:
        w, c = (int(v) for v in g.split("x"))
    except ValueError:
        w, c = 8, 24
    return (w, c) if (w, c) in ((4, 16), (8, 24), (8, 48)) else (8, 24)


def split_tables(plan, uni_kind: int, act: int = 1):
    t = tables(plan, uni_kind, act)
    if t is None:
        return None
    wide = t["WAVES"] != 8
    if wide and os.environ.get("ZUKO_AMD_SPLIT_WIDE", "1") == "0":
        return None
    cached = getattr(plan, "_split_cache", None)
    if cached is not None and cached[0] == (uni_kind, act, split_geometry()):
        return cached[1]
    NH, HT, NIT = t["NH"], t["HT"], t["NIT"]
    tm = plan.fine_tilemask
    n_otg, n_itile = tm.shape[1], tm.shape[2]
    waves, ch = (4, 24) if wide else split_geometry()
    B_OT, B_IP, NB, BASE, blocks_of = [], [], [], [], []
    cursor = 0

    def pair_block(fg, t0, t1):
        idx = -np.ones((64, 8), dtype=np.int64)
        if t0 is not None:
            idx[:, :4] = fg[t0]
        if t1 is not None:
            idx[:, 4:] = fg[t1]
        return idx

    for l in range(NH):
        fg = plan.fine_gather[l].reshape(-1, 64, 4)
        pos, k = {}, 0
        for otg in range(n_otg):
            for it in range(n_itile):
                m = int(tm[l, otg, it])
                for b in range(4):
                    if m >> b & 1:
                        pos[(otg * 4 + b, it)] = k
                        k += 1
        n_in = NIT if l == 0 else HT[l - 1]
        blocks = []
        for ot in range(HT[l]):
            for ip in range(-(-n_in // 2)):
                t0, t1 = pos.get((ot, 2 * ip)), pos.get((ot, 2 * ip + 1))
                if t0 is None and t1 is None:
                    continue
                blocks.append(pair_block(fg, t0, t1))
                B_OT.append(ot), B_IP.append(ip)
        NB.append(len(blocks))
        BASE.append(cursor)
        cursor += 3 * len(blocks)
        blocks_of.append(blocks)
    nt = plan.layout.nt
    fg = plan.fine_gather[NH].reshape(-1, 64, 4)
    G_IP, GOFFP, blocks, k = [], [0], [], 0
    for g in range(t["NG"]):
        its = t["G_IT"][t["GOFF"][g] : t["GOFF"][g + 1]]
        at = {it: k + i * nt for i, it in enumerate(its)}
        k += len(its) * nt
        for ip in sorted({it // 2 for it in its}):
            for b in range(nt):
                t0, t1 = at.get(2 * ip), at.get(2 * ip + 1)
                blocks.append(pair_block(fg, None if t0 is None else t0 + b, None if t1 is None else t1 + b))
            G_IP.append(ip)
        GOFFP.append(len(G_IP))
    last_base = cursor
    cursor += 3 * len(blocks)
    n_chunks = -(-cursor // ch)
    pad_blocks = -(-(n_chunks * ch - cursor) // 3)
    blocks_of.append(blocks + [-np.ones((64, 8), dtype=np.int64)] * pad_blocks)
    stream_images = max(n_chunks * ch, cursor + 3 * pad_blocks)
    gathers = [np.stack(b).astype(np.int32).reshape(-1) if b else np.zeros(0, np.int32) for b in blocks_of]
    out = dict(t)
    for key in ("S_OTG", "S_IT", "S_MASK", "NS", "GOFF", "G_IT"):
        out.pop(key)
    nr = 2 if ch == 48 else 3
    per_cu = 2 if (waves == 4 and not wide) else 1
    xlds = int(t["D"] % 4 == 0 and (nr * ch * 256 + (t["BIAS_STRIDE"] * NH + t["NG"] * nt * 16) + 1024 + 256 + waves * 16 * (((t["D"] + 3) // 4) * 4 + 4)) * 4 * per_cu <= 160 * 1024)
    out.update({"split": 1, "TMAX": int(2 * -(-t["TMAX"] // 2)), "NB": NB, "B_OT": B_OT, "B_IP": B_IP, "BASE": BASE, "LAST_BASE": last_base, "GOFF": GOFFP, "G_IP": G_IP, "NCHUNK": n_chunks, "STREAM_IMAGES": stream_images,
                "WAVES": waves, "CH": ch, "NR": nr, "XLDS": xlds, "OCC": 1 if wide else 2})
    plan._split_cache = ((uni_kind, act, split_geometry()), (out, gathers))
    return out, gathers


def half_enabled() -> bool:
    from . import fused

    return split_enabled() and fused.matmul_precision() == "f16x2"


def half_tables(plan, uni_kind: int, act: int = 1):
    ts = split_tables(plan, uni_kind, act)
    if ts is None:
        return None
    t, gathers = ts
    if t["WAVES"] != 8 or t["NH"] > 3 or uni_kind in SPLIT_ONLY_KINDS or t["CH"] != 24:
        return None
    cached = getattr(plan, "_half_cache", None)
    if cached is not None and cached[0] == (uni_kind, act):
        return cached[1]
    ch, NH, nt = t["CH"], t["NH"], plan.layout.nt
    n_last = t["GOFF"][-1] * nt
    cursor = 2 * (sum(t["NB"]) + n_last)
    n_chunks = -(-cursor // ch)
    pad_blocks = -(-(n_chunks * ch - cursor) // 2)
    last = gathers[NH][: n_last * 512]
    g = [np.asarray(x) for x in gathers[:NH]] + [np.concatenate([last, -np.ones(pad_blocks * 512, dtype=np.int32)]).astype(np.int32)]
    out = {k: v for k, v in t.items() if k not in ("split", "TRAIN_OK")}
    bias_floats = plan.bias_off[-1] + len(plan.bias_gather[-1])
    rows = t["WAVES"] * 16 * (((t["D"] + 3) // 4) * 4 + 4) if t["XLDS"] else 0
    nr = 4 if (4 * ch * 256 + bias_floats + 1024 + 256 + rows) * 4 <= 160 * 1024 else 3
    out.update({"half": 1, "BASE": [2 * sum(t["NB"][:l]) for l in range(NH)], "LAST_BASE": 2 * sum(t["NB"]), "NCHUNK": n_chunks, "STREAM_IMAGES": max(n_chunks * ch, cursor + 2 * pad_blocks),
                "NR": nr, "IMAGES": cursor, "BPOS": HALF_BPOS, "TRAIN_OK": 0})
    plan._half_cache = ((uni_kind, act), (out, g))
    return out, g


HALF_LOOK = 1
HALF_BPOS = 8


def half_trigger(t: dict, c: int) -> int:
    ch = t["CH"]
    last = min(t["IMAGES"], (c + 1) * ch) - 1
    return min(c * ch + t["BPOS"] + 1, last)


def half_schedule(t: dict) -> tuple:
    ch, nr, per, look = t["CH"], t["NR"], t["CH"] // t["WAVES"], HALF_LOOK
    nit, last_base, images = t["NIT"], t["LAST_BASE"], t["IMAGES"]
    pro = [("issue",)] * (nr - 1) + [("x", nit), ("wait", 0, True), ("barrier",)]
    if nr == 4:
        trig = {half_trigger(t, c): c for c in range(t["NCHUNK"])}
        xpos = min((p for p in trig if p >= last_base), default=-1)
    else:
        xpos = -(-last_base // ch) * ch
    ev = []

    def read(pos):
        if nr != 4 and pos % ch == 0:
            ev.extend([("wait", (nr - 2) * per + (nit if pos == xpos else 0), True), ("barrier",), ("issue",)])
        ev.append(("read", pos))
        if nr == 4 and pos in trig:
            ev.extend([("wait", nit if pos == xpos else 0, pos % ch != t["BPOS"] + 1), ("barrier",), ("issue",)])

    def layer(base, nb, last_of):
        lk = min(look, nb)
        for b in range(lk):
            read(base + 2 * b), read(base + 2 * b + 1)
        for s in range(nb):
            if s + lk < nb:
                read(base + 2 * (s + lk)), read(base + 2 * (s + lk) + 1)
            ahead = lk if s + lk < nb else nb - 1 - s
            ev.append(("settle", (2 if s + lk < nb else 0) if last_of(s) else 2 * ahead))

    off = 0
    for l in range(t["NH"]):
        nb = t["NB"][l]
        ots = t["B_OT"][off : off + nb]
        layer(t["BASE"][l], nb, lambda s: s + 1 == nb or ots[s + 1] != ots[s])
        off += nb
    ev.append(("x", nit))
    nbl = (images - last_base) // 2
    nt = nbl // max(t["GOFF"][-1], 1)
    ends = {g1 * nt - 1 for g1 in t["GOFF"][1:]}
    layer(last_base, nbl, lambda s: s in ends)
    return pro, ev




def _split(t: dict):
    n0 = t["NS"][0]
    core = {k: v for k, v in t.items() if k != "S_IT"}
    core["S_IT_rest"] = t["S_IT"][n0:]
    return core, t["S_IT"][:n0]


def _digest(obj) -> str:
    return hashlib.sha256(json.dumps(obj, sort_keys=True).encode()).hexdigest()[:16]


def _arr(name: str, ctype: str, vals) -> str:
    vals = list(vals) or [0]
    return f"  static constexpr {ctype} {name}[{len(vals)}] = {{{', '.join(str(int(v)) for v in vals)}}};"


def _pick(t: dict, *names) -> dict:
    return {n: t[n] for n in names}


@dataclasses.dataclass(frozen=True)
class Family:

    prefix: str
    header: str
    stamp: object
    shape: tuple
    prefix_sums: dict
    entry: str
    params: tuple
    launcher: str
    sig: object
    index: object
    meta: object


_FORWARD = dict(entry="zk_ars_launch", params=(("const zk::ArArgs*", "a"), ("int", "abi"), ("int", "args_bytes"), ("int", "train"), ("void*", "stream")))
_BACKWARD = dict(entry="zk_ars_dgrad_launch", params=(("const zk::ArArgs*", "a"), ("int", "abi"), ("int", "args_bytes"), ("void*", "stream")))

ARS = Family(
    prefix="ars", header="fused_ar_static_impl.h", stamp=_header_digest, **_FORWARD, launcher="zk::ars_launch<Shape, {uni}>",
    shape=(("int", ("D", "DIN", "NIT", "NH", "TMAX", "NG", "NCHUNK")), ("int", ("BIAS_STRIDE", "LAST_BASE", "WAVES", "ACT")), ("bool", ("XLDS", "HAS_ALT", "TRAIN_OK")),
           ("int[]", ("HT", "NS", "BASE")), ("unsigned char[]", ("S_OTG", "S_IT", "S_ALT", "S_MASK")), ("int[]", ("GOFF",)), ("unsigned char[]", ("G_IT",))),
    prefix_sums={"NS": "SOFF"},
    sig=lambda t, alt: {"core": _split(t)[0], "l0": _split(t)[1], "alt": alt},
    index=lambda t: _digest(_split(t)[0]),
    meta=lambda t: _pick(t, "uni", "ACT", "D", "DIN", "HT", "WAVES", "TRAIN_OK", "XLDS"),
)
ARX = Family(
    prefix="arx", header="fused_ar_split_impl.h", stamp=_header_digest, **_FORWARD, launcher="zk::arx_launch<Shape, {uni}>",
    shape=(("int", ("D", "DIN", "NIT", "NH", "TMAX", "NG", "NCHUNK")), ("int", ("BIAS_STRIDE", "LAST_BASE", "WAVES", "CH", "NR", "ACT", "OCC")),
           ("bool", ("XLDS", "HAS_ALT=false", "TRAIN_OK")), ("int[]", ("HT", "NB", "BASE")), ("unsigned char[]", ("B_OT", "B_IP")), ("int[]", ("GOFF",)), ("unsigned char[]", ("G_IP",))),
    prefix_sums={"NB": "BOFF"},
    sig=lambda t, alt: {"split": t},
    index=lambda t: "x" + _digest(t),
    meta=lambda t: dict(_pick(t, "uni", "ACT", "D", "DIN", "HT", "WAVES", "CH", "TRAIN_OK", "XLDS", "NCHUNK"), split=1),
)
ARH = dataclasses.replace(
    ARX, prefix="arh", header="fused_ar_half_impl.h", stamp=_half_digest, launcher="zk::arh_launch<Shape, {uni}>",
    shape=ARX.shape[:2] + (("int", ("IMAGES", "BPOS")), ("bool", ("XLDS",))) + ARX.shape[3:],
    sig=lambda t, alt: {"half": t},
    index=lambda t: "h" + _digest(t),
    meta=lambda t: dict(_pick(t, "uni", "ACT", "D", "DIN", "HT", "WAVES", "CH", "TRAIN_OK", "XLDS", "NCHUNK"), half=1, split=2),
)
ARSD_F32 = Family(
    prefix="arsd", header="fused_ar_static_impl.h", stamp=_header_digest, **_BACKWARD, launcher="zk::ars_dgrad_launch<Shape>",
    shape=(("int", ("DIN", "DOUT", "NIT", "NH", "TMAX", "NCHUNK", "WAVES=8", "ACT=1")), ("bool", ("HAS_ALT=false",)), ("int[]", ("HT", "NS", "BASE")),
           ("unsigned char[]", ("S_OTG", "S_IT", "S_ALT", "S_MASK"))),
    prefix_sums={"NS": "SOFF"},
    sig=lambda t, alt: {"t": t},
    index=None,
    meta=lambda t: _pick(t, "DIN", "DOUT", "HT"),
)
ARSD_SPLIT = dataclasses.replace(
    ARSD_F32, header="fused_ar_split_impl.h", launcher="zk::arxd_launch<Shape>",
    shape=(("int", ("DIN0", "DOUT", "NH", "TMAX", "NCHUNK", "WAVES=8", "CH", "NP0", "ACT=1")), ("int[]", ("HT", "NB", "BASE")), ("unsigned char[]", ("P0", "B_OT", "B_IP"))),
    prefix_sums={"NB": "BOFF"},
    meta=lambda t: {"DIN": t["DIN0"], "DOUT": t["DOUT"], "HT": t["HT"]},
)
ARSD_FULL = dataclasses.replace(
    ARSD_SPLIT, launcher="zk::arxb_launch<Shape, {uni}>", shape=ARSD_SPLIT.shape + (("int", ("NG",)), ("int[]", ("PB",))))
FAMILIES = {"ars": ARS, "arx": ARX, "arh": ARH, "arsd": {1: ARSD_F32, 2: ARSD_SPLIT, 3: ARSD_FULL}}


def emit(fam: Family, t: dict, alt: list | None = None) -> str:
    v = dict(t, HAS_ALT=alt is not None)
    if "S_IT" in t:
        n0 = t["NS"][0]
        v["S_ALT"] = (alt if alt is not None else t["S_IT"][:n0]) + t["S_IT"][n0:]
    lines = ["// generated by zuko_amd/static_ar.py — do not edit", f'#include "{fam.header}"', "namespace {", "struct Shape {"]
    for ctype, names in fam.shape:
        if ctype.endswith("[]"):
            for name in names:
                lines.append(_arr(name, ctype[:-2], v[name]))
                if name in fam.prefix_sums:
                    lines.append(_arr(fam.prefix_sums[name], "int", [sum(v[name][:i]) for i in range(len(v[name]) + 1)]))
        else:
            show = (lambda x: "true" if x else "false") if ctype == "bool" else str
            lines.append(f"  static constexpr {ctype} " + ", ".join(n.replace("=", " = ") if "=" in n else f"{n} = {show(v[n])}" for n in names) + ";")
    launcher = fam.launcher.format(uni=UNI_TYPES.get(t.get("uni")))
    lines += [
        "};",
        "}  // namespace",
        f'extern "C" int {fam.entry}({", ".join(f"{c} {n}" for c, n in fam.params)}) {{ return {launcher}({", ".join(n for _, n in fam.params)}); }}',
        "",
    ]
    return "\n".join(lines)


def _identity(fam: Family, t: dict, alt: list | None = None):
    stamp = fam.stamp()
    ident = fam.sig(t, alt)
    stem = f"{fam.prefix}_{_digest(dict(ident, headers=stamp))}"
    meta = {"so": stem + ".so", "core": "chain" if fam.index is None else fam.index(t), "l0": ident.get("l0", []), "alt": alt, "headers": stamp, **fam.meta(t)}
    return stem, meta




class StaticKernel:

    def __init__(self, so: str, meta: dict, entry: str) -> None:
        self.so, self.meta = so, meta
        self.cdll = ctypes.CDLL(so)
        self.launcher = ctypes.cast(getattr(self.cdll, entry), ctypes.c_void_p)


_LOCK = threading.Lock()
_LOADED: dict[str, StaticKernel] = {}
_INDEX: dict | None = None


def _scan() -> dict:
    global _INDEX
    idx: dict = {}
    for d in _dirs():
        try:
            names = sorted(os.listdir(d)) if os.path.isdir(d) else []
        except OSError:
            names = []
        for name in names:
            if name.endswith(".json"):
                try:
                    with open(os.path.join(d, name)) as f:
                        meta = json.load(f)
                except (OSError, ValueError):
                    continue
                if meta.get("headers") == _stamp_of(meta) and os.path.exists(os.path.join(d, meta["so"])):
                    meta["dir"] = d
                    idx.setdefault(meta["core"], []).append(meta)
    _INDEX = idx
    return idx


def _torch_lib_dir() -> str:
    import importlib.util

    spec = importlib.util.find_spec("torch")
    return os.path.join(os.path.dirname(spec.origin), "lib")


def compile_unit(fam: Family, t: dict, alt: list | None = None, verbose: bool = False, out_dir: str | None = None) -> dict | None:
    stem, meta = _identity(fam, t, alt)
    so = _build_so(stem, lambda: emit(fam, t, alt), meta, verbose, out_dir)
    if so is None:
        return None
    global _INDEX
    _INDEX = None
    return dict(meta, dir=os.path.dirname(so))


def _load(meta: dict, entry: str = _FORWARD["entry"]) -> StaticKernel | None:
    k = _LOADED.get(meta["so"])
    if k is None:
        so = os.path.join(meta.get("dir", ARS_DIR), meta["so"])
        try:
            k = StaticKernel(so, meta, entry)
        except OSError as exc:
            _warn_once("load:" + so, f"cannot load {so}: {exc}")
            return None
        _LOADED[meta["so"]] = k
    return k


def _found(fam: Family, t: dict, l0: list | None):
    if fam.index is None:
        name = _identity(fam, t)[0] + ".so"
        so = _LOADED[name].so if name in _LOADED else _find(name)
        return None if so is None else ({"so": name, "dir": os.path.dirname(so)}, 0)
    idx = _INDEX if _INDEX is not None else _scan()
    for meta in idx.get(fam.index(t), []):
        if l0 is None or meta["l0"] == l0:
            return meta, 0
        if meta["alt"] is not None and meta["alt"] == l0:
            return meta, 1
    return None


def find_or_compile(fam: Family, t: dict, allow: bool, l0: list | None = None, verbose: bool = False, out_dir: str | None = None):
    with _LOCK:
        found = _found(fam, t, l0)
    if found is None and allow:
        meta = compile_unit(fam, t, None, verbose, out_dir)
        found = None if meta is None else (meta, 0)
    if found is None:
        return None
    with _LOCK:
        k = _load(found[0], fam.entry)
    return None if k is None else (k, found[1])


def _enabled() -> bool:
    return os.environ.get("ZUKO_AMD_NO_STATIC_AR", "0") != "1"


def jit_enabled() -> bool:
    return os.environ.get("ZUKO_AMD_JIT", "1") != "0" and _hipcc() is not None


def jit_min_rows() -> int:
    try:
        return int(os.environ.get("ZUKO_AMD_JIT_MIN_ROWS", str(1 << 15)))
    except ValueError:
        return 1 << 15


def _jit_allowed(rows: int | None) -> bool:
    return rows is not None and rows >= jit_min_rows() and jit_enabled()


def _jit_verbose() -> bool:
    return os.environ.get("ZUKO_AMD_JIT_VERBOSE", "0") == "1"


JIT_CUMULATIVE_FACTOR = 8
# ... 129 lines not shown
            ok = (a_ < in_l) & (b_ < out_l) & (row >= 0)
            return np.where(ok, row * in_l + np.asarray(cols[l])[np.minimum(a_, in_l - 1)], -1)

        def live(ot, ip):
            return bool(M[ip * 32 : ip * 32 + 32, ot * 16 : ot * 16 + 16].any())

        order = [(ot, ip) for ip in range(n_ip) for ot in range(n_ot)] if c == 0 else [(ot, ip) for ot in range(n_ot) for ip in range(n_ip)]
        blocks = []
        for ot, ip in order:
            if live(ot, ip):
                blocks.append(block(ot, ip))
                B_OT.append(ot), B_IP.append(ip)
                if c == 0 and (not P0 or P0[-1] != ip):
                    P0.append(ip)
        if not blocks:
            return None
        NB.append(len(blocks))
        BASE.append(cursor)
        cursor += 3 * len(blocks)
        blocks_of.append(blocks)
    n_chunks = -(-cursor // ch)
    pad = -(-(n_chunks * ch - cursor) // 3)
    blocks_of[-1] = blocks_of[-1] + [-np.ones((64, 8), dtype=np.int64)] * pad
    t = {"chain": 2, "DIN0": int(masks_sorted[-1].shape[0]), "DOUT": int(din), "NH": n, "HT": HT, "TMAX": int(2 * -(-max(HT) // 2)), "NB": NB, "BASE": BASE, "B_OT": B_OT, "B_IP": B_IP,
         "NP0": len(P0), "P0": P0, "NCHUNK": n_chunks, "STREAM_IMAGES": max(n_chunks * ch, cursor + 3 * pad), "WAVES": 8, "CH": ch}
    if t["TMAX"] > 16:
        return None
    if packed is not None:
        n_pairs = t["DIN0"] // 32
        ips = np.asarray(B_IP[: NB[0]])
        t.update({"chain": 3, "uni": int(packed["uni"]), "NG": ng, "NT": nt, "PB": [int((ips < pp).sum()) for pp in range(n_pairs + 1)], "MODROW": [int(r) for r in mod_row]})
    return t, [np.stack(b).astype(np.int32).reshape(-1) for b in blocks_of]


def chain_kernel(t: dict, allow_compile: bool):
    found = find_or_compile(FAMILIES["arsd"][t["chain"]], t, allow_compile)
    return None if found is None else found[0]



PREBUILT = [
    ("rqs", 64, 0, (256, 256, 256), 8),
    ("affine", 64, 0, (256, 256, 256), 0),
    ("rqs", 3, 5, (128, 128, 128), 8),
    ("rqs", 32, 0, (512, 512), 8),
    ("rqs", 32, 0, (256, 256), 8),
    ("affine", 16, 0, (128, 128), 0),
    ("rqs", 20, 3, (100, 72), 8),
    ("affine", 7, 2, (40,), 0),
    ("rqs", 24, 8, (384, 512, 320), 8),
    ("rqs", 16, 2, (64, 64), 8, "ELU"),
    ("affine", 12, 0, (48, 32), 0, "Tanh"),
    ("rqs", 64, 0, (256, 256, 256), 16),
    ("affine", 12, 0, (64, 64), 0),
    ("rqs", 128, 0, (256, 256, 256), 8), ("rqs", 64, 8, (256, 256), 8), ("rqs", 16, 0, (512, 512, 512), 8),
    ("sos", 4, 2, (32, 32), 0), ("bern", 4, 2, (32, 32), 0), ("sos", 64, 0, (256, 256, 256), 0), ("bern", 64, 0, (256, 256, 256), 0),
]


def _plans_for(kind: str, features: int, context: int, hidden, bins: int, activation: str | None = None):
    import torch

    from . import fused
    from .flows.autoregressive import MaskedAutoregressiveTransform
    from .nn import MaskedLinear
    from .transforms import BoundedBernsteinTransform, MonotonicAffineTransform, MonotonicRQSTransform, ShiftedSOSPolynomialTransform

    out = []
    for order in (torch.arange(features), torch.flipud(torch.arange(features))):
        if kind == "affine":
            t = MaskedAutoregressiveTransform(features, context, order=order, hidden_features=list(hidden), univariate=MonotonicAffineTransform, shapes=[(), ()])
            layout = fused.uni_layout("affine", 2)
        elif kind == "sos":
            t = MaskedAutoregressiveTransform(features, context, order=order, hidden_features=list(hidden), univariate=ShiftedSOSPolynomialTransform, shapes=[(3, 5), ()])
            layout = fused.uni_layout("sos", 16)
        elif kind == "bern":
            t = MaskedAutoregressiveTransform(features, context, order=order, hidden_features=list(hidden), univariate=BoundedBernsteinTransform, shapes=[(17,)])
            layout = fused.uni_layout("bern", 17)
        else:
            t = MaskedAutoregressiveTransform(features, context, order=order, hidden_features=list(hidden), univariate=MonotonicRQSTransform, shapes=[(bins,), (bins,), (bins - 1,)])
            layout = fused.uni_layout("rqs", 3 * bins - 1, bins)
        masks = [m.mask for m in t.hyper if isinstance(m, MaskedLinear)]
        wide = max(list(hidden) + [features + context]) > fused.MAX_WIDTH
        out.append((fused.build_plan(masks, features, layout, max_width=fused.MAX_WIDTH_WIDE if wide else fused.MAX_WIDTH), layout, [m for m in t.hyper if isinstance(m, MaskedLinear)]))
    return out


def chain_tables_for(lins, full: bool = False, packed: dict | None = None):
    import torch

    from .train import SortedPlan

    sp = SortedPlan(lins, 1, torch.device("cpu"))
    n = len(lins)
    if n < 2 or n > 4 or any(m is None for m in sp.mask_s_cpu):
        return None
    if full:
        return chain_split_tables(sp.mask_s_cpu, sp.rows_cpu, sp.cols_cpu, packed=packed) if (packed is not None or sp.shapes[-1][0] % 4 == 0) else None
    return chain_tables(sp.mask_s_cpu[: n - 1], sp.rows_cpu[: n - 1], sp.cols_cpu[: n - 1])


def prebuild(verbose: bool = True, jobs: int = 4) -> list[str]:
    from concurrent.futures import ThreadPoolExecutor

    if os.path.isdir(ARS_DIR):
        for name in os.listdir(ARS_DIR):
            if name.endswith(".json"):
                try:
                    with open(os.path.join(ARS_DIR, name)) as f:
                        m_ = json.load(f)
                        stale = m_.get("headers") != _stamp_of(m_)
                except (OSError, ValueError):
                    stale = True
                if stale:
                    for ext in (".json", ".so", ".hip"):
                        try:
                            os.remove(os.path.join(ARS_DIR, name[: -len(".json")] + ext))
                        except OSError:
                            pass
            elif name.startswith(".lock_"):
                try:
                    os.remove(os.path.join(ARS_DIR, name))
                except OSError:
                    pass
    work = []

    def want(fam, t, alt=None):
        if (fam, t, alt) not in work:
            work.append((fam, t, alt))

    for entry in PREBUILT:
        kind, features, context, hidden, bins = entry[:5]
        import torch

        from .nn import _act_code

        act = _act_code(getattr(torch.nn, entry[5])()) if len(entry) > 5 else 1
        (pa, layout, lins_a), (pd, _, lins_d) = _plans_for(kind, features, context, hidden, bins)
        if act == 1:
            for lins, pl in ((lins_a, pa), (lins_d, pd)):
                cands = [chain_tables_for(lins), chain_tables_for(lins, full=True)]
                if (features + context) % 4 == 0 and layout.kind in (0, 1) and layout.total in (2, 23) and pl is not None:
                    cands.append(chain_tables_for(lins, full=True, packed={"uni": layout.kind, "featmap": pl.featmap, "nt": layout.nt, "fpl": layout.fpl, "total": layout.total}))
                for tg in cands:
                    if tg is not None:
                        want(FAMILIES["arsd"][tg[0]["chain"]], tg[0])
        for pl in (pa, pd):
            ts = split_tables(pl, layout.kind, act)
            if ts is not None:
                want(ARX, ts[0])
            th = half_tables(pl, layout.kind, act)
            if th is not None:
                want(ARH, th[0])
        if layout.kind in SPLIT_ONLY_KINDS:
            continue
        ta, td = tables(pa, layout.kind, act), tables(pd, layout.kind, act)
        if ta is None or td is None:
            raise RuntimeError(f"zuko_amd.static_ar: no static kernel for the prebuilt shape {entry}")
        (ca, la), (cdesc, ld) = _split(ta), _split(td)
        if ca == cdesc:
            want(ARS, ta, None if la == ld else ld)
        else:
            want(ARS, ta), want(ARS, td)
    prev = os.environ.get("ZUKO_AMD_SPLIT_GEOM")
    if prev is None:
        os.environ["ZUKO_AMD_SPLIT_GEOM"] = "4x16"
        try:
            kind, features, context, hidden, bins = PREBUILT[0][:5]
            for pl, layout, _ in _plans_for(kind, features, context, hidden, bins):
                pl._split_cache = None
                ts = split_tables(pl, layout.kind, 1)
                if ts is not None:
                    want(ARX, ts[0])
        finally:
            del os.environ["ZUKO_AMD_SPLIT_GEOM"]
    with ThreadPoolExecutor(max_workers=jobs) as ex:
        metas = list(ex.map(lambda w: compile_unit(*w, verbose, ARS_DIR), work))
    if any(m is None for m in metas):
        raise RuntimeError("zuko_amd.static_ar: a prebuilt static kernel failed to compile")
    return [m["so"] for m in metas]


if __name__ == "__main__":
    sys.path.insert(0, os.path.dirname(HERE))
    import zuko_amd.static_ar as me

    print("\n".join(me.prebuild()))
```

zuko_amd/transforms.py:

```python

from __future__ import annotations

from typing import Callable, Sequence

import torch
from torch import Tensor
from torch.distributions import Transform, constraints
from torch.distributions.utils import _sum_rightmost

from . import ops

__all__ = [
    "AdditiveTransform",
    "AutoregressiveTransform",
    "BernsteinTransform",
    "BoundedBernsteinTransform",
    "CircularShiftTransform",
    "ComposedTransform",
    "CouplingTransform",
    "DependentTransform",
    "FreeFormJacobianTransform",
    "GaussianizationTransform",
    "MonotonicAffineTransform",
    "MonotonicNetworkTransform",
# ... 233 lines not shown

    def __init__(self, bound: float = 1.0, **kwargs) -> None:
        super().__init__(**kwargs)
        self.bound = bound
        self.domain = constraints.interval(-bound, bound)
        self.codomain = constraints.interval(-bound, bound)

    def __repr__(self) -> str:
        return f"{self.__class__.__name__}(bound={self.bound})"

    def _call(self, x):
        return torch.remainder(x, 2 * self.bound) - self.bound

    def _inverse(self, y):
        return torch.remainder(y, 2 * self.bound) - self.bound

    def log_abs_det_jacobian(self, x, y):
        return torch.zeros_like(x)


class AdditiveTransform(Transform):

    domain = constraints.real
    codomain = constraints.real
    bijective = True
    sign = +1

    def __init__(self, shift: Tensor, **kwargs) -> None:
        super().__init__(**kwargs)
        self.shift = shift

    def _call(self, x):
        return x + self.shift

    def _inverse(self, y):
        return y - self.shift

    def log_abs_det_jacobian(self, x, y):
        return torch.zeros_like(x)




class DependentTransform(Transform):

    def __init__(self, base: Transform, reinterpreted: int, **kwargs) -> None:
        super().__init__(**kwargs)
        self.base = base
        self.reinterpreted = reinterpreted

    def __repr__(self) -> str:
        return f"{self.__class__.__name__}({self.base}, {self.reinterpreted})"

    @property
    def domain(self):
        return constraints.independent(self.base.domain, self.reinterpreted)

    @property
    def codomain(self):
        return constraints.independent(self.base.codomain, self.reinterpreted)

    @property
    def bijective(self) -> bool:
        return self.base.bijective

    def _call(self, x):
        return self.base(x)

    @property
    def inv(self) -> Transform:
        return DependentTransform(self.base.inv, self.reinterpreted)

    def _inverse(self, y):
        return self.base.inv(y)

    def log_abs_det_jacobian(self, x, y):
        return self.call_and_ladj(x)[1] if hasattr(self.base, "call_and_ladj_reduced") and self.reinterpreted == 1 else _sum_rightmost(
            self.base.log_abs_det_jacobian(x, y), self.reinterpreted
        )

    def call_and_ladj(self, x):
        if self.reinterpreted == 1 and hasattr(self.base, "call_and_ladj_reduced") and x.dim() >= 1:
            return self.base.call_and_ladj_reduced(x)
        y, ladj = self.base.call_and_ladj(x)
        return y, _sum_rightmost(ladj, self.reinterpreted)

    def forward_shape(self, shape):
        return self.base.forward_shape(shape)

    def inverse_shape(self, shape):
        return self.base.inverse_shape(shape)


class ComposedTransform(Transform):

    def __init__(self, *transforms: Transform, **kwargs) -> None:
        super().__init__(**kwargs)
        if not transforms:
            raise AssertionError("'transforms' cannot be empty")
        self.transforms = list(transforms)
        dim = 0
        for t in reversed(self.transforms):
            dim = t.domain.event_dim + max(dim - t.codomain.event_dim, 0)
        self.domain_dim = dim
        for t in self.transforms:
            dim += t.codomain.event_dim - t.domain.event_dim
        self.codomain_dim = dim

    def __repr__(self) -> str:
        body = "\n".join(f"  ({i}): " + repr(t).replace("\n", "\n  ") for i, t in enumerate(self.transforms))
        return f"{self.__class__.__name__}(\n{body}\n)"

    @staticmethod
    def _lift(c, extra: int):
        return constraints.independent(c, extra) if extra > 0 else c

    @property
    def domain(self):
        d = self.transforms[0].domain
        return self._lift(d, self.domain_dim - d.event_dim)

    @property
    def codomain(self):
        c = self.transforms[-1].codomain
        return self._lift(c, self.codomain_dim - c.event_dim)

    @property
    def bijective(self) -> bool:
        return all(t.bijective for t in self.transforms)

    def _call(self, x):
        for t in self.transforms:
            x = t(x)
        return x

    @property
    def inv(self) -> Transform:
        rev = ComposedTransform.__new__(ComposedTransform)
        Transform.__init__(rev)
        rev.transforms = [t.inv for t in reversed(self.transforms)]
        rev.domain_dim, rev.codomain_dim = self.codomain_dim, self.domain_dim
        return rev

    def _inverse(self, y):
        for t in reversed(self.transforms):
            y = t.inv(y)
        return y

    def log_abs_det_jacobian(self, x, y):
        return self.call_and_ladj(x)[1]

    def call_and_ladj(self, x, base=None):
        dim = self.domain_dim
        total = None
        owned = False
        last = self.transforms[-1]
        for t in self.transforms:
            if base is not None and t is last and (owned or total is None) and dim == t.domain.event_dim == t.codomain.event_dim == 1:
                term = getattr(t, "call_and_log_prob", None)
                lp = term(x, total, *base) if term is not None else None
                if lp is not None:
                    return None, lp
            acc = getattr(t, "call_and_accumulate_ladj", None)
            y = acc(x, total) if (acc is not None and owned and dim == t.domain.event_dim) else None
            if y is not None:
                x = y
            else:
                x, ladj = t.call_and_ladj(x)
                ladj = _sum_rightmost(ladj, dim - t.domain.event_dim)
                owned = acc is not None if total is None else True
                total = ladj if total is None else total + ladj
            dim += t.codomain.event_dim - t.domain.event_dim
        return x, total

    def forward_shape(self, shape):
        for t in self.transforms:
            shape = t.forward_shape(shape)
        return shape

    def inverse_shape(self, shape):
        for t in reversed(self.transforms):
            shape = t.inverse_shape(shape)
        return shape


class AutoregressiveTransform(Transform):

    domain = constraints.real_vector
    codomain = constraints.real_vector
    bijective = True

    def __init__(self, meta: Callable[[Tensor], Transform], passes: int, **kwargs) -> None:
        super().__init__(**kwargs)
        self.meta = meta
        self.passes = passes

    def _call(self, x):
        return self.meta(x)(x)

    def _inverse(self, y):
        x = torch.zeros_like(y)
        for _ in range(self.passes):
            x = self.meta(x).inv(y)
        return x

    def log_abs_det_jacobian(self, x, y):
        return self.meta(x).log_abs_det_jacobian(x, y)

    def call_and_ladj(self, x):
        return self.meta(x).call_and_ladj(x)


class CouplingTransform(Transform):

    domain = constraints.real_vector
    codomain = constraints.real_vector
    bijective = True

    def __init__(self, meta: Callable[[Tensor], Transform], mask: Tensor, **kwargs) -> None:
        super().__init__(**kwargs)
        self.meta = meta
        self.idx_a = mask.nonzero().squeeze(-1)
        self.idx_b = (~mask).nonzero().squeeze(-1)

    def split(self, x):
        return x[..., self.idx_a], x[..., self.idx_b]

    def merge(self, a, b, shape):
        out = a.new_empty(shape)
        out[..., self.idx_a] = a
        out[..., self.idx_b] = b
        return out

    def _call(self, x):
        a, b = self.split(x)
        return self.merge(a, self.meta(a)(b), x.shape)

    def _inverse(self, y):
        a, b = self.split(y)
        return self.merge(a, self.meta(a).inv(b), y.shape)

    def log_abs_det_jacobian(self, x, y):
        a, b = self.split(x)
        return self.meta(a).log_abs_det_jacobian(b, self.split(y)[1])

    def call_and_ladj(self, x):
        a, b = self.split(x)
        yb, ladj = self.meta(a).call_and_ladj(b)
        return self.merge(a, yb, x.shape), ladj


class FreeFormJacobianTransform(Transform):

    domain = constraints.real_vector
    codomain = constraints.real_vector
    bijective = True

    def __init__(self, f: Callable[[Tensor, Tensor], Tensor], t0=0.0, t1=1.0, phi=(), atol: float = 1e-6, rtol: float = 1e-5, exact: bool = True,
                 kernel=None, **kwargs) -> None:
        super().__init__(**kwargs)
        self.f = f
        self.t0 = t0
        self.t1 = t1
        self.phi = tuple(p for p in phi if p.requires_grad)
        self.atol = atol
        self.rtol = rtol
        self.exact = exact
        self.kernel = kernel
        self.trace_scale = 1e-2

    def _integrate(self, x: Tensor, t0, t1, with_ladj: bool):
        ops._require_device(x)
        if self.kernel is None or (with_ladj and not self.exact):
            return None
        module, c = self.kernel
        return ops.cnf_integrate(module, c, x, float(t0), float(t1), self.atol, self.rtol, self.trace_scale, with_ladj, self.phi)

    def _call(self, x: Tensor) -> Tensor:
        out = self._integrate(x, self.t0, self.t1, False)
        if out is not None:
            return out[0]
        from .utils import odeint

        ops.CNF_STATS.clear()
        ops.CNF_STATS.update(path="torch")
        return odeint(self.f, x, self.t0, self.t1, self.phi, self.atol, self.rtol)

    @property
    def inv(self) -> Transform:
        return FreeFormJacobianTransform(self.f, self.t1, self.t0, self.phi, self.atol, self.rtol, self.exact, kernel=self.kernel)

    def _inverse(self, y: Tensor) -> Tensor:
        return self.inv._call(y)

    def log_abs_det_jacobian(self, x: Tensor, y: Tensor) -> Tensor:
        return self.call_and_ladj(x)[1]

    def augmented(self, x: Tensor, eps: Tensor | None = None):
        graph = torch.is_grad_enabled() and (x.requires_grad or bool(self.phi))
        if self.exact:
            seeds = torch.eye(x.shape[-1], dtype=x.dtype, device=x.device).expand(*x.shape, -1).movedim(-1, 0)
        elif eps is None:
            eps = torch.randn_like(x)

        def system(t: Tensor, x: Tensor, ladj: Tensor):
            with torch.enable_grad():
# ... 23 lines not shown
```

Before: 78.56 million samples/s.

## Fuse all autoregressive transforms of a flow into one persistent kernel launch

Adds a flow-level kernel variant that runs all T autoregressive transforms in one launch. Each sample's row stays in LDS between transforms, and ladj plus the base log-prob term are accumulated in registers. Per-transform biases are DMA'd into LDS from inside the weight ring, near the end of each pass, and alternating input-permutation tables handle the two transform orderings. This removes the per-transform kernel launches and the global-memory round trips of the intermediate x/y and ladj tensors, at the cost of more complex ring synchronisation and a new JIT kernel family.

```diff
diff --git a/include/zuko_amd.h b/include/zuko_amd.h
--- a/include/zuko_amd.h
+++ b/include/zuko_amd.h
@@ -134,6 +134,11 @@
   uint32_t* amax3;
   const void* base_loc;
   const void* base_scale;
+  int32_t flow_transforms;
+  int32_t flow_bias_stride;
+  int32_t flow_featmaps;
+  int32_t pad2_;
+  const void* flow_table;
 } zk_ar_args_v1;
 
 int zk_ar_forward(const zk_ar_args_v1* args, void* stream);
diff --git a/zuko_amd/csrc/fused_ar.hip b/zuko_amd/csrc/fused_ar.hip
--- a/zuko_amd/csrc/fused_ar.hip
+++ b/zuko_amd/csrc/fused_ar.hip
@@ -512,9 +512,33 @@
   return ar_launch_v1(part, false, p, stream);
 }
 
+static int ar_flow_launch(const zk_ar_args_v1* p, void* stream) {
+  if (p->N < 0 || p->N > 0x7fffffff || p->D < 4 || p->D > 256 || p->D % 4 || p->DIN != p->D || p->ldx % 4 || ((uintptr_t)p->x % 16) || p->n_chunks < 1 || p->n_layers < 2) return ZK_EINVAL;
+  if (p->n_groups * 8 > ArLds::FMAP_WORDS || (p->base_loc != nullptr) != (p->base_scale != nullptr) || !p->ladj || p->accumulate || p->rev || p->bin_out || p->knots_out) return ZK_EINVAL;
+  if (p->wdescale0 != 0.0 || p->wdescale1 != 0.0 || p->wdescale2 != 0.0 || p->wdescale3 != 0.0) return ZK_EINVAL;
+  if (p->N == 0) return 0;
+  ArArgs a{};
+  a.N = p->N; a.D = p->D; a.DIN = p->D;
+  a.x = (const float*)p->x; a.ldx = p->ldx;
+  a.y = (float*)p->y; a.ldy = p->ldy; a.ladj = (float*)p->ladj;
+  a.stream = (const float*)p->wstream;
+  a.L = p->n_layers; a.NG = p->n_groups; a.n_chunks = p->n_chunks; a.act = p->act; a.bias_floats = p->bias_floats;
+  a.bound = (float)p->bound; a.ls = (float)log(p->slope);
+  a.lc = rqs_lean_const(p->bound, log(p->slope));
+  a.g0 = 0; a.g1 = p->n_groups;
+  for (int l = 0; l < 8; ++l) a.olim[l] = 3;
+  a.eps = 1e-6f;
+  a.base_loc = (const float*)p->base_loc; a.base_scale = (const float*)p->base_scale;
+  ArhFlow f{};
+  f.T = p->flow_transforms; f.bias_stride = p->flow_bias_stride; f.n_fmaps = p->flow_featmaps;
+  f.bias = (const float*)p->bias; f.featmap = p->featmap; f.table = (const float*)p->flow_table;
+  return ((arhf_launch_fn)p->launcher)(&a, &f, ARS_ABI, (int)sizeof(ArArgs), (int)sizeof(ArhFlow), stream);
+}
+
 int zk_ar_forward_static(const zk_ar_args_v1* args, void* stream) {
   zk_ar_args_v1 args_norm_;
   if (!AR_ARGS_OK(args) || !args->launcher) return ZK_EINVAL;
+  if (args->flow_transforms != 0) return args->flow_transforms > 0 ? ar_flow_launch(args, stream) : ZK_EINVAL;
   ArPartial part;
   part.static_fn = args->launcher; part.rev = args->rev;
   part.gl_nodes01 = args->gl_nodes01; part.gl_weights01 = args->gl_weights01; part.eps = args->eps;
diff --git a/zuko_amd/csrc/fused_ar_half_impl.h b/zuko_amd/csrc/fused_ar_half_impl.h
--- a/zuko_amd/csrc/fused_ar_half_impl.h
+++ b/zuko_amd/csrc/fused_ar_half_impl.h
@@ -111,7 +111,7 @@
   }
 };
 
-template <int WAVES, int CH, int IMAGES, int BPOS> struct ArhRing4 {
+template <int WAVES, int CH, int IMAGES, int BPOS, bool FLOW = false> struct ArhRing4 {
   static constexpr int NR = 4, PER = CH / WAVES, PIVOT = PER > 4 ? 4 : 0, CHB = CH * AR_TF * 4, NCH = (IMAGES + CH - 1) / CH;
   static_assert(PER * WAVES == CH && PER <= 6 && BPOS % 2 == 0 && BPOS >= 2 * (ARH_LOOK + 1) && BPOS + 1 < CH && CH % 2 == 0 && IMAGES % 2 == 0, "ring geometry");
   static constexpr int trigger(int c) {
@@ -131,6 +131,14 @@
   unsigned lane_off;
   unsigned lane16;
   unsigned cur_off;
+  bool rows_in_flight;
+  const char* bias_src;
+  char* bias_dst;
+  int bias_n, wave_id;
+  __device__ __forceinline__ void bias_request() {
+    for (int p = wave_id; p < bias_n; p += WAVES)
+      __builtin_amdgcn_global_load_lds((const __attribute__((address_space(1))) void*)(bias_src + p * 1024 + (size_t)lane16), (__attribute__((address_space(3))) void*)(bias_dst + p * 1024), 16, 0, 0);
+  }
   __device__ __forceinline__ void start(float* lds, const float* stream, int n_chunks, int wave, int lane) {
     const int b0 = wave * PER + PIVOT;
     gsrc = reinterpret_cast<const char*>(stream + b0 * AR_TF);
@@ -138,6 +146,7 @@
     goff = 0; gend = (unsigned)n_chunks * CHB; fill_off = 0;
     lane16 = (unsigned)lane * 16;
     lane_off = (unsigned)(size_t)((__attribute__((address_space(3))) float*)lds) + lane16;
+    if constexpr (FLOW) { wave_id = wave; rows_in_flight = false; bias_n = 0; }
 #pragma unroll
     for (int i = 0; i < NR - 1; ++i) issue();
     read_off = (NR - 1) * CHB;
@@ -155,9 +164,17 @@
     goff = (goff + CHB == gend) ? 0 : goff + CHB;
     fill_off = (fill_off + CHB == NR * CHB) ? 0 : fill_off + CHB;
   }
-  template <int XV, bool DRAIN> __device__ __forceinline__ void boundary() {
+  template <int XV, bool DRAIN> __device__ __forceinline__ void wait() {
     if constexpr (DRAIN) asm volatile("s_waitcnt vmcnt(%0) lgkmcnt(0)" ::"n"(XV) : "memory");
     else asm volatile("s_waitcnt vmcnt(%0)" ::"n"(XV) : "memory");
+  }
+  template <int XV, bool DRAIN> __device__ __forceinline__ void boundary() {
+    if constexpr (FLOW && XV != 0) {
+      if (rows_in_flight) wait<XV, DRAIN>();
+      else wait<0, DRAIN>();
+    } else {
+      wait<XV, DRAIN>();
+    }
     if (ARX_ABL != 4) __builtin_amdgcn_s_barrier();
     asm volatile("" ::: "memory");
     issue();
@@ -177,11 +194,18 @@
       asm volatile("ds_read_b128 %0, %1 offset:%2" : "=v"(v) : "v"(cur_off), "n"((S % CH) * AR_TF * 4));
     }
     if constexpr (S == trigger(S / CH)) boundary<XV, (S % CH != BPOS + 1)>();
+    if constexpr (FLOW && NCH >= 2) {
+      if constexpr (S == trigger(NCH - 2)) bias_request();
+    }
     return v;
   }
 };
 
-template <class S, int L, class Ring> __device__ __forceinline__ void arh_hidden(Ring& ring, const float* bias_q, const ArhB (&in)[S::TMAX / 2], f32x4 (&out)[S::TMAX], float d) {
+template <class S, int L, bool ALT> constexpr int arh_ip(int s) {
+  if constexpr (ALT) return S::B_IP_ALT[s];
+  else return ArxPat<S>::ip(L, s);
+}
+template <class S, int L, class Ring, bool ALT = false> __device__ __forceinline__ void arh_hidden(Ring& ring, const float* bias_q, const ArhB (&in)[S::TMAX / 2], f32x4 (&out)[S::TMAX], float d) {
   typedef ArxPat<S> P;
   constexpr int NB = S::NB[L], BASE = S::BASE[L], HTL = S::HT[L];
   ars_for<HTL>([&](auto t_) ARS_ALWAYS_INLINE {
@@ -199,7 +223,8 @@
       ars_for<2>([&](auto p) ARS_ALWAYS_INLINE { a[b][p] = ring.template read<BASE + 2 * b + decltype(p)::value>(); });
     });
     ars_for<NB>([&](auto s_) ARS_ALWAYS_INLINE {
-      constexpr int s = s_, ot = P::ot(L, s), ip = P::ip(L, s), cur = s % (LOOK + 1);
+      constexpr int s = s_, ot = P::ot(L, s), cur = s % (LOOK + 1);
+      constexpr int ip = arh_ip<S, L, ALT>(s);
       constexpr bool first_of_tile = (s == 0 || P::ot(L, s - 1) != ot), last_of_tile = (s + 1 == NB || P::ot(L, s + 1) != ot);
       if constexpr (first_of_tile) acc = f32x4{0.f, 0.f, 0.f, 0.f};
       if constexpr (last_of_tile) bs = arx_lds_raw<ot * 64>(bias_addr);
@@ -229,10 +254,16 @@
   }
 }
 
-template <class S, int L, class Ring> __device__ __forceinline__ void arh_hidden_stack(Ring& ring, const float* bias_lds, int q, ArhB (&in)[S::TMAX / 2], f32x4 (&out)[S::TMAX], const ArArgs& a,
-                                                                                       float& inv_s, float& poison) {
+template <class S, int L, class Ring, bool HAS_ALT = false> __device__ __forceinline__ void arh_hidden_stack(Ring& ring, const float* bias_lds, int q, ArhB (&in)[S::TMAX / 2], f32x4 (&out)[S::TMAX], const float* wd,
+                                                                                                         float& inv_s, float& poison, bool alt = false) {
   if constexpr (L < S::NH) {
-    arh_hidden<S, L>(ring, bias_lds + L * S::BIAS_STRIDE + 4 * q, in, out, a.wdescale[L] * inv_s);
+    if constexpr (HAS_ALT && L == 0) {
+      static_assert(S::BASE[0] == 0, "B_IP_ALT lists the first layer's blocks");
+      if (alt) arh_hidden<S, L, Ring, true>(ring, bias_lds + L * S::BIAS_STRIDE + 4 * q, in, out, wd[L] * inv_s);
+      else arh_hidden<S, L, Ring>(ring, bias_lds + L * S::BIAS_STRIDE + 4 * q, in, out, wd[L] * inv_s);
+    } else {
+      arh_hidden<S, L, Ring>(ring, bias_lds + L * S::BIAS_STRIDE + 4 * q, in, out, wd[L] * inv_s);
+    }
     constexpr int HTL = S::HT[L];
     float amax = 0.f;
     if constexpr (S::ACT == 1 && ARH_EPI_PINNED) {
@@ -268,19 +299,199 @@
     const f32x4 zero = {0.f, 0.f, 0.f, 0.f};
 #pragma unroll
     for (int p = 0; p < (HTL + 1) / 2; ++p) arh_split(out[2 * p], 2 * p + 1 < HTL ? out[2 * p + 1] : zero, s, in[p]);
-    arh_hidden_stack<S, L + 1, Ring>(ring, bias_lds, q, in, out, a, inv_s, poison);
-  }
+    arh_hidden_stack<S, L + 1, Ring, HAS_ALT>(ring, bias_lds, q, in, out, wd, inv_s, poison, alt);
+  }
+}
+
+template <typename Uni> __device__ __forceinline__ void arh_flow_epilogue(float (&p)[4 * Uni::NT], const ArArgs& a, const int (&fid)[Uni::FPL], const float (&xin)[Uni::FPL], float poison, float* xr,
+                                                                          const float* base, int D, bool term, float& lacc) {
+  constexpr int FPL = Uni::FPL, TOTAL = Uni::TOTAL;
+#pragma unroll
+  for (int fi = 0; fi < FPL; ++fi) Uni::template poison<false>(p, fi * TOTAL, poison);
+  auto ld = [&](int i) { return p[i]; };
+#pragma unroll
+  for (int fi = 0; fi < FPL; ++fi) {
+    const int f = fid[fi];
+    if (f >= 0) {
+      float yv, lj;
+      Uni::fwd(ld, fi * TOTAL, a, xin[fi], yv, lj);
+      lacc += lj;
+      if (term) {
+        const float df = yv - base[f];
+        lacc += __builtin_fmaf(-(df * df), base[D + f], base[2 * D + f]);
+      } else {
+        xr[f] = yv;
+      }
+    }
+  }
+}
+
+template <class S, typename Uni, bool DIAG, bool TERM, bool FLOW, class Ring, class XReq, class Fids>
+__device__ __forceinline__ void arh_pass(const ArArgs& a, Ring& ring, XReq& x_request, f32x4 (&xnext)[S::NIT], float* bias_lds, const Fids& fids, float* xr, const float* base, const ArLane& ln,
+                                         int64_t tile, const float* wd, bool first, bool last, bool term, float& total, bool alt = false) {
+  constexpr bool RING4 = S::NR == 4;
+  static_assert(!FLOW || (RING4 && S::XLDS && S::DIN == S::D && !DIAG && !TERM), "flow pass: four-slot ring, rows in LDS, no context columns");
+  constexpr int NT = Uni::NT, FPL = Uni::FPL, WAVES = S::WAVES;
+  constexpr int NG = S::NG;
+  constexpr int NSTEP = S::GOFF[NG];
+  constexpr bool XLDS = S::XLDS;
+  const int wave = ln.wave, j = ln.j, q = ln.q;
+  const float* bias_last = bias_lds + S::NH * S::BIAS_STRIDE;
+  const unsigned bias_last_addr = arx_lds_addr(bias_last + 4 * q);
+  if constexpr (FLOW) {
+    asm volatile("" ::: "memory");
+    __builtin_amdgcn_wave_barrier();
+  }
+  const int64_t n = tile * (16 * WAVES) + wave * 16 + j;
+  const bool live = n < a.N;
+  const int64_t nc = live ? n : a.N - 1;
+  const float* xrow = a.x + nc * a.ldx;
+
+  ArhB in[S::TMAX / 2];
+  f32x4 out[S::TMAX];
+  float poison;
+  float inv_s;
+  {
+    f32x4 xin[S::NIT + 1];
+#pragma unroll
+    for (int it = 0; it < S::NIT; ++it) {
+      f32x4 v = {0.f, 0.f, 0.f, 0.f};
+      if constexpr (FLOW) {
+        if ((it + 1) * 16 <= S::DIN || it * 16 + 4 * q < S::DIN) v = *reinterpret_cast<const f32x4*>(xr + it * 16 + 4 * q);
+      } else if (ARH_PREFETCH) {
+        if ((it + 1) * 16 <= S::DIN || it * 16 + 4 * q < S::DIN) v = xnext[it];
+      } else {
+        if ((it + 1) * 16 <= S::DIN || it * 16 + 4 * q < S::DIN) v = *reinterpret_cast<const f32x4*>(xrow + it * 16 + 4 * q);
+      }
+      xin[it] = v;
+    }
+    xin[S::NIT] = f32x4{0.f, 0.f, 0.f, 0.f};
+    poison = ar_poison_of<S::NIT>(xin);
+    float amax = 0.f;
+#pragma unroll
+    for (int it = 0; it < S::NIT; ++it)
+#pragma unroll
+      for (int r = 0; r < 4; ++r) amax = fmaxf(amax, fabsf(xin[it][r]));
+    if constexpr (XLDS && !FLOW) ar_rows_in<S::D>(xr, q, xin);
+    float s;
+    arh_scale(amax, s, inv_s);
+    if constexpr (S::ACT == 1 && ARH_EPI_PINNED) {
+      if (!(amax < ARH_AMAX_OVERFLOW)) poison = __builtin_nanf("");
+    }
+#pragma unroll
+    for (int p = 0; p < (S::NIT + 1) / 2; ++p) arh_split(xin[2 * p], xin[2 * p + 1], s, in[p]);
+  }
+
+  float ladj_in = 0.f;
+  if constexpr (!FLOW) {
+    if (ARH_PREFETCH && a.ladj && a.accumulate && live && q == 0) ladj_in = a.ladj[n];
+  }
+
+  if constexpr (FLOW) arh_hidden_stack<S, 0, Ring, S::FLOW_ALT>(ring, bias_lds, q, in, out, wd, inv_s, poison, alt);
+  else arh_hidden_stack<S, 0, Ring>(ring, bias_lds, q, in, out, wd, inv_s, poison);
+
+  const float dl = wd[S::NH] * inv_s;
+  float lacc = 0.f;
+  constexpr int NBL = NSTEP * NT;
+  constexpr int LOOKL = ARH_LOOK < NBL ? ARH_LOOK : NBL;
+  f32x4 w[LOOKL + 1][2];
+  constexpr int XPOS = []() constexpr {
+    if constexpr (!ARH_PREFETCH) return -1;
+    else if constexpr (RING4) return Ring::first_trigger_from(S::LAST_BASE);
+    else return (S::LAST_BASE + S::CH - 1) / S::CH * S::CH;
+  }();
+  if constexpr (FLOW) {
+    asm volatile("" ::: "memory");
+    if (last) {
+      x_request(tile + gridDim.x < a.n_tiles ? tile + gridDim.x : tile, xnext);
+    } else {
+#pragma unroll
+      for (int it = 0; it < S::NIT; ++it) asm("" : "=v"(xnext[it]));
+    }
+    ring.rows_in_flight = last;
+    asm volatile("" ::: "memory");
+  } else if (ARH_PREFETCH) {
+    asm volatile("" ::: "memory");
+    x_request(tile + gridDim.x < a.n_tiles ? tile + gridDim.x : tile, xnext);
+    asm volatile("" ::: "memory");
+  }
+#define ARH_READ_LAST(POS) ring.template read<(POS), ((POS) == XPOS ? S::NIT : 0)>()
+  ars_for<LOOKL>([&](auto b_) ARS_ALWAYS_INLINE {
+    constexpr int b = b_;
+    ars_for<2>([&](auto p) ARS_ALWAYS_INLINE { w[b][p] = ARH_READ_LAST(S::LAST_BASE + 2 * b + decltype(p)::value); });
+  });
+  ars_for<NG>([&](auto g_) ARS_ALWAYS_INLINE {
+    constexpr int g = g_, ST0 = S::GOFF[g], GN = S::GOFF[g + 1] - S::GOFF[g];
+    int fid[FPL];
+    float xin[FPL];
+    fids.template fetch<XLDS>(g, xr, xrow, fid, xin);
+    float bv[3 * FPL];
+    if constexpr (TERM && !FLOW) fids.fetch_base(fid, base, S::D, bv);
+    f32x4 acc[NT], bs[NT];
+    if constexpr (GN == 0) {
+      const float* bg = bias_last + (g * NT) * 16 + 4 * q;
+      ars_for<NT>([&](auto t) ARS_ALWAYS_INLINE { bs[t] = *reinterpret_cast<const f32x4*>(bg + t * 16); });
+    }
+    ars_for<NT>([&](auto t) ARS_ALWAYS_INLINE { acc[t] = f32x4{0.f, 0.f, 0.f, 0.f}; });
+    ars_for<GN>([&](auto i_) ARS_ALWAYS_INLINE {
+      constexpr int st = ST0 + decltype(i_)::value, ip = S::G_IP[st];
+      ars_for<NT>([&](auto t_) ARS_ALWAYS_INLINE {
+        constexpr int t = t_, blk = st * NT + t, cur = blk % (LOOKL + 1);
+        constexpr bool last_of_group = (decltype(i_)::value == GN - 1 && t == NT - 1);
+        if constexpr (last_of_group) {
+          ars_for<NT>([&](auto u) ARS_ALWAYS_INLINE { bs[u] = arx_lds_raw<(g * NT + decltype(u)::value) * 64>(bias_last_addr); });
+        }
+        if constexpr (blk + LOOKL < NBL) {
+          constexpr int nx = (blk + LOOKL) % (LOOKL + 1);
+          ars_for<2>([&](auto p) ARS_ALWAYS_INLINE { w[nx][p] = ARH_READ_LAST(S::LAST_BASE + 2 * (blk + LOOKL) + decltype(p)::value); });
+        }
+        constexpr int ahead = (blk + LOOKL < NBL ? LOOKL : NBL - 1 - blk);
+        if constexpr (last_of_group) arh_settle<(blk + LOOKL < NBL ? 2 : 0)>(w[cur][0], w[cur][1]);
+        else arh_settle<2 * ahead>(w[cur][0], w[cur][1]);
+        if constexpr (last_of_group) {
+#pragma unroll
+          for (int u = 0; u < NT; ++u) arh_touch(bs[u]);
+        }
+        if (ARX_FENCE) __builtin_amdgcn_sched_barrier(0);
+        arh_block(w[cur], in[ip], acc[t]);
+        if (ARX_FENCE) __builtin_amdgcn_sched_barrier(0);
+      });
+    });
+    float p[4 * NT];
+    ars_for<NT>([&](auto t) ARS_ALWAYS_INLINE {
+#pragma unroll
+      for (int r = 0; r < 4; ++r) {
+        p[4 * t + r] = __builtin_fmaf(acc[t][r], dl, bs[t][r]);
+        if (ARH_POISON_ONE) asm("" : "+v"(p[4 * t + r]));
+      }
+    });
+    if constexpr (FLOW) arh_flow_epilogue<Uni>(p, a, fid, xin, poison, xr, base, S::D, last && term, lacc);
+    else ar_uni_epilogue<Uni, DIAG, XLDS, true, TERM>(p, a, fid, xin, poison, xr, n, live, S::D, lacc, bv);
+  });
+#undef ARH_READ_LAST
+  if constexpr (FLOW) {
+    lacc += __shfl_xor(lacc, 16, 64);
+    lacc += __shfl_xor(lacc, 32, 64);
+    total = first ? lacc : total + lacc;
+    if (last) {
+      if (live && q == 0) a.ladj[n] = total;
+      if (!term) ar_rows_out<S::D>(xr, q, a.y + n * a.ldy, live);
+    }
+    return;
+  }
+  if (ARH_PREFETCH) ar_ladj_store<true>(a, lacc, n, live, q, ladj_in);
+  if constexpr (XLDS && !TERM) ar_rows_out<S::D>(xr, q, a.y + n * a.ldy, live);
+  if (!ARH_PREFETCH) ar_ladj_store(a, lacc, n, live, q);
 }
 
 template <class S, typename Uni, bool DIAG, bool TERM> __device__ __forceinline__ void arh_body(const ArArgs& a) {
   constexpr bool RING4 = S::NR == 4;
   typedef std::conditional_t<RING4, ArhRing4<S::WAVES, S::CH, S::IMAGES, S::BPOS>, ArhRing<S::WAVES, S::CH, S::NR>> Ring;
   static_assert(S::WAVES == 8 && (S::NR == 3 || S::NR == 4) && S::TMAX <= 16 && S::TMAX % 2 == 0 && S::OCC == 2, "two-part split kernels: widths <= 256, two wavefronts per SIMD");
-  constexpr int NT = Uni::NT, FPL = Uni::FPL, TOTAL = Uni::TOTAL, WAVES = S::WAVES;
+  constexpr int NT = Uni::NT, FPL = Uni::FPL, WAVES = S::WAVES;
   constexpr int NG = S::NG;
   constexpr int NSTEP = S::GOFF[NG];
   static_assert(S::IMAGES == S::LAST_BASE + 2 * NSTEP * NT && (S::IMAGES + S::CH - 1) / S::CH == S::NCHUNK, "stream length");
-  constexpr bool XLDS = S::XLDS;
   const ArLane ln;
   const int tid = ln.tid, lane = ln.lane, wave = ln.wave, j = ln.j, q = ln.q;
 
@@ -315,126 +526,11 @@
   float* const base = ArLds::base(fmap_lds, NG * 4 * FPL);
   if constexpr (TERM) ArLds::stage_base<64 * WAVES>(a, tid, base, S::D);
   ArLds::stage<64 * WAVES>(a, tid, bias_lds, fmap_lds, NG * 4 * FPL);
-  const float* bias_last = bias_lds + S::NH * S::BIAS_STRIDE;
-  const unsigned bias_last_addr = arx_lds_addr(bias_last + 4 * q);
   const ArFids<NG, FPL, (NG * FPL <= 32)> fids(fmap_lds, q);
 
-  for (int64_t tile = blockIdx.x; tile < a.n_tiles; tile += gridDim.x) {
-    const int64_t n = tile * (16 * WAVES) + wave * 16 + j;
-    const bool live = n < a.N;
-    const int64_t nc = live ? n : a.N - 1;
-    const float* xrow = a.x + nc * a.ldx;
-
-    ArhB in[S::TMAX / 2];
-    f32x4 out[S::TMAX];
-    float poison;
-    float inv_s;
-    {
-      f32x4 xin[S::NIT + 1];
-#pragma unroll
-      for (int it = 0; it < S::NIT; ++it) {
-        f32x4 v = {0.f, 0.f, 0.f, 0.f};
-        if (ARH_PREFETCH) {
-          if ((it + 1) * 16 <= S::DIN || it * 16 + 4 * q < S::DIN) v = xnext[it];
-        } else {
-          if ((it + 1) * 16 <= S::DIN || it * 16 + 4 * q < S::DIN) v = *reinterpret_cast<const f32x4*>(xrow + it * 16 + 4 * q);
-        }
-        xin[it] = v;
-      }
-      xin[S::NIT] = f32x4{0.f, 0.f, 0.f, 0.f};
-      poison = ar_poison_of<S::NIT>(xin);
-      float amax = 0.f;
-#pragma unroll
-      for (int it = 0; it < S::NIT; ++it)
-#pragma unroll
-        for (int r = 0; r < 4; ++r) amax = fmaxf(amax, fabsf(xin[it][r]));
-      if constexpr (XLDS) ar_rows_in<S::D>(xr, q, xin);
-      float s;
-      arh_scale(amax, s, inv_s);
-      if constexpr (S::ACT == 1 && ARH_EPI_PINNED) {
-        if (!(amax < ARH_AMAX_OVERFLOW)) poison = __builtin_nanf("");
-      }
-#pragma unroll
-      for (int p = 0; p < (S::NIT + 1) / 2; ++p) arh_split(xin[2 * p], xin[2 * p + 1], s, in[p]);
-    }
-
-    float ladj_in = 0.f;
-    if (ARH_PREFETCH && a.ladj && a.accumulate && live && q == 0) ladj_in = a.ladj[n];
-
-    arh_hidden_stack<S, 0, Ring>(ring, bias_lds, q, in, out, a, inv_s, poison);
-
-    const float dl = a.wdescale[S::NH] * inv_s;
-    float lacc = 0.f;
-    constexpr int NBL = NSTEP * NT;
-    constexpr int LOOKL = ARH_LOOK < NBL ? ARH_LOOK : NBL;
-    f32x4 w[LOOKL + 1][2];
-    constexpr int XPOS = []() constexpr {
-      if constexpr (!ARH_PREFETCH) return -1;
-      else if constexpr (RING4) return Ring::first_trigger_from(S::LAST_BASE);
-      else return (S::LAST_BASE + S::CH - 1) / S::CH * S::CH;
-    }();
-    if (ARH_PREFETCH) {
-      asm volatile("" ::: "memory");
-      x_request(tile + gridDim.x < a.n_tiles ? tile + gridDim.x : tile, xnext);
-      asm volatile("" ::: "memory");
-    }
-#define ARH_READ_LAST(POS) ring.template read<(POS), ((POS) == XPOS ? S::NIT : 0)>()
-    ars_for<LOOKL>([&](auto b_) ARS_ALWAYS_INLINE {
-      constexpr int b = b_;
-      ars_for<2>([&](auto p) ARS_ALWAYS_INLINE { w[b][p] = ARH_READ_LAST(S::LAST_BASE + 2 * b + decltype(p)::value); });
-    });
-    ars_for<NG>([&](auto g_) ARS_ALWAYS_INLINE {
-      constexpr int g = g_, ST0 = S::GOFF[g], GN = S::GOFF[g + 1] - S::GOFF[g];
-      int fid[FPL];
-      float xin[FPL];
-      fids.template fetch<XLDS>(g, xr, xrow, fid, xin);
-      float bv[3 * FPL];
-      if constexpr (TERM) fids.fetch_base(fid, base, S::D, bv);
-      f32x4 acc[NT], bs[NT];
-      if constexpr (GN == 0) {
-        const float* bg = bias_last + (g * NT) * 16 + 4 * q;
-        ars_for<NT>([&](auto t) ARS_ALWAYS_INLINE { bs[t] = *reinterpret_cast<const f32x4*>(bg + t * 16); });
-      }
-      ars_for<NT>([&](auto t) ARS_ALWAYS_INLINE { acc[t] = f32x4{0.f, 0.f, 0.f, 0.f}; });
-      ars_for<GN>([&](auto i_) ARS_ALWAYS_INLINE {
-        constexpr int st = ST0 + decltype(i_)::value, ip = S::G_IP[st];
-        ars_for<NT>([&](auto t_) ARS_ALWAYS_INLINE {
-          constexpr int t = t_, blk = st * NT + t, cur = blk % (LOOKL + 1);
-          constexpr bool last_of_group = (decltype(i_)::value == GN - 1 && t == NT - 1);
-          if constexpr (last_of_group) {
-            ars_for<NT>([&](auto u) ARS_ALWAYS_INLINE { bs[u] = arx_lds_raw<(g * NT + decltype(u)::value) * 64>(bias_last_addr); });
-          }
-          if constexpr (blk + LOOKL < NBL) {
-            constexpr int nx = (blk + LOOKL) % (LOOKL + 1);
-            ars_for<2>([&](auto p) ARS_ALWAYS_INLINE { w[nx][p] = ARH_READ_LAST(S::LAST_BASE + 2 * (blk + LOOKL) + decltype(p)::value); });
-          }
-          constexpr int ahead = (blk + LOOKL < NBL ? LOOKL : NBL - 1 - blk);
-          if constexpr (last_of_group) arh_settle<(blk + LOOKL < NBL ? 2 : 0)>(w[cur][0], w[cur][1]);
-          else arh_settle<2 * ahead>(w[cur][0], w[cur][1]);
-          if constexpr (last_of_group) {
-#pragma unroll
-            for (int u = 0; u < NT; ++u) arh_touch(bs[u]);
-          }
-          if (ARX_FENCE) __builtin_amdgcn_sched_barrier(0);
-          arh_block(w[cur], in[ip], acc[t]);
-          if (ARX_FENCE) __builtin_amdgcn_sched_barrier(0);
-        });
-      });
-      float p[4 * NT];
-      ars_for<NT>([&](auto t) ARS_ALWAYS_INLINE {
-#pragma unroll
-        for (int r = 0; r < 4; ++r) {
-          p[4 * t + r] = __builtin_fmaf(acc[t][r], dl, bs[t][r]);
-          if (ARH_POISON_ONE) asm("" : "+v"(p[4 * t + r]));
-        }
-      });
-      ar_uni_epilogue<Uni, DIAG, XLDS, true, TERM>(p, a, fid, xin, poison, xr, n, live, S::D, lacc, bv);
-    });
-#undef ARH_READ_LAST
-    if (ARH_PREFETCH) ar_ladj_store<true>(a, lacc, n, live, q, ladj_in);
-    if constexpr (XLDS && !TERM) ar_rows_out<S::D>(xr, q, a.y + n * a.ldy, live);
-    if (!ARH_PREFETCH) ar_ladj_store(a, lacc, n, live, q);
-  }
+  float unused = 0.f;
+  for (int64_t tile = blockIdx.x; tile < a.n_tiles; tile += gridDim.x)
+    arh_pass<S, Uni, DIAG, TERM, false>(a, ring, x_request, xnext, bias_lds, fids, xr, base, ln, tile, a.wdescale, true, true, TERM, unused);
   asm volatile("s_waitcnt vmcnt(0)" ::: "memory");
 }
 
@@ -469,4 +565,90 @@
   return ar_launch_dyn_lds(fn, 256, 64 * S::WAVES, lds, a, stream);
 }
 
-}
+template <class S, typename Uni> __device__ __forceinline__ void arhf_body(const ArArgs& a, const ArhFlow& f) {
+  typedef ArhRing4<S::WAVES, S::CH, S::IMAGES, S::BPOS, true> Ring;
+  static_assert(S::WAVES == 8 && S::NR == 4 && S::TMAX <= 16 && S::TMAX % 2 == 0 && S::OCC == 2 && S::NCHUNK >= 2, "flow kernel: the four-slot two-part geometry, two chunks or more per pass");
+  constexpr int NT = Uni::NT, FPL = Uni::FPL, WAVES = S::WAVES, NG = S::NG, NFM = NG * 4 * FPL;
+  static_assert(S::IMAGES == S::LAST_BASE + 2 * S::GOFF[NG] * NT && (S::IMAGES + S::CH - 1) / S::CH == S::NCHUNK, "stream length");
+  const ArLane ln;
+  const int tid = ln.tid, lane = ln.lane, wave = ln.wave, j = ln.j, q = ln.q;
+
+  Ring ring;
+  ring.start(ars_lds, a.stream, f.T * a.n_chunks, wave, lane);
+  auto x_request = [&](int64_t tile, f32x4 (&xv)[S::NIT]) ARS_ALWAYS_INLINE {
+    const int64_t n = tile * (16 * WAVES) + wave * 16 + j;
+    const float* row = a.x + (n < a.N ? n : a.N - 1) * a.ldx;
+#pragma unroll
+    for (int it = 0; it < S::NIT; ++it) {
+      const int col = it * 16 + 4 * q;
+      xv[it] = *reinterpret_cast<const f32x4*>(row + ((it + 1) * 16 <= S::DIN || col < S::DIN ? col : S::DIN - 4));
+    }
+  };
+  f32x4 xnext[S::NIT];
+  x_request(blockIdx.x, xnext);
+
+  float* const bias_lds = ars_lds + S::NR * S::CH * AR_TF;
+  int* const fmap_lds = ArLds::fmap(bias_lds, 2 * f.bias_stride);
+  float* const xr = ArLds::row(fmap_lds, wave, j, a.xs);
+  float* const base = ArLds::base(fmap_lds, f.n_fmaps * NFM);
+  if (f.term) ArLds::stage_base<64 * WAVES>(a, tid, base, S::D);
+  for (int i = tid; i < a.bias_floats; i += 64 * WAVES) bias_lds[i] = f.bias[i];
+  for (int i = tid; i < f.n_fmaps * NFM; i += 64 * WAVES) fmap_lds[i] = f.featmap[i];
+  __syncthreads();
+  ring.bias_n = f.bias_stride / 256;
+  const __attribute__((address_space(4))) float* const table = (const __attribute__((address_space(4))) float*)f.table;
+
+  int buf = 0;
+  for (int64_t tile = blockIdx.x; tile < a.n_tiles; tile += gridDim.x) {
+    ar_rows_in<S::D>(xr, q, xnext);
+    float total = 0.f;
+#pragma unroll 1
+    for (int t = 0; t < f.T; ++t) {
+      float wd[4];
+#pragma unroll
+      for (int l = 0; l < 4; ++l) wd[l] = table[t * 8 + l];
+      const int fm = __builtin_bit_cast(int, table[t * 8 + 4]);
+      const bool alt = __builtin_bit_cast(int, table[t * 8 + 5]) != 0;
+      const int tn = t + 1 == f.T ? 0 : t + 1;
+      ring.bias_src = reinterpret_cast<const char*>(f.bias + (size_t)tn * f.bias_stride);
+      ring.bias_dst = reinterpret_cast<char*>(bias_lds + (buf ^ 1) * f.bias_stride);
+      const ArFids<NG, FPL, (NG * FPL <= 32)> fids(fmap_lds + fm * NFM, q);
+      arh_pass<S, Uni, false, false, true>(a, ring, x_request, xnext, bias_lds + buf * f.bias_stride, fids, xr, base, ln, tile, wd, t == 0, t + 1 == f.T, f.term != 0, total, alt);
+      buf ^= 1;
+    }
+  }
+  asm volatile("s_waitcnt vmcnt(0)" ::: "memory");
+}
+
+template <class S, typename Uni> __global__ __launch_bounds__(64 * S::WAVES, S::OCC) void arhf_kernel(ArArgs a, ArhFlow f) { arhf_body<S, Uni>(a, f); }
+
+template <class S, typename Uni> static int arhf_launch(const ArArgs* in, const ArhFlow* fin, int abi, int args_bytes, int flow_bytes, void* stream) {
+  if (abi != ARS_ABI || args_bytes != (int)sizeof(ArArgs) || flow_bytes != (int)sizeof(ArhFlow)) return ZK_EINVAL;
+  if constexpr (S::NR != 4 || !S::XLDS || S::DIN != S::D || S::D % 4 != 0 || S::NCHUNK < 2) {
+    return ZK_EINVAL;
+  } else {
+    ArArgs a = *in;
+    ArhFlow f = *fin;
+    if (a.D != S::D || a.DIN != S::DIN || a.L != S::NH + 1 || a.act != S::ACT || a.sched || a.NG != S::NG || a.n_chunks != S::NCHUNK || a.l1rev) return ZK_EINVAL;
+    if (f.T < 1 || f.T > 64 || f.n_fmaps < 1 || f.n_fmaps > f.T || f.bias_stride % 256 || f.bias_stride < a.bias_floats || !f.bias || !f.featmap || !f.table) return ZK_EINVAL;
+    if (!a.x || !a.stream || !a.ladj || a.accumulate || a.bin_out || a.knots_out) return ZK_EINVAL;
+    a.n_tiles = (a.N + 16 * S::WAVES - 1) / (16 * S::WAVES);
+    a.xs = ((S::D + 3) / 4) * 4 + 4;
+    f.term = a.base_loc != nullptr;
+    if (f.term ? !a.base_scale : (!a.y || a.ldy % 4 != 0 || (uintptr_t)a.y % 16 != 0)) return ZK_EINVAL;
+    if (f.n_fmaps * S::NG * 4 * Uni::FPL + (f.term ? 3 * S::D : 0) > ArLds::FMAP_WORDS) return ZK_EINVAL;
+    a.xlds = 1;
+    const int lds = ArLds::bytes(S::NR * S::CH * AR_TF, 2 * f.bias_stride, S::WAVES, a.xs);
+    if (lds > 160 * 1024) return ZK_EINVAL;
+    const void* fn = (const void*)arhf_kernel<S, Uni>;
+    hipError_t e = grant_dyn_lds(fn, lds);
+    if (e != hipSuccess) return (int)e;
+    const unsigned grid = (unsigned)(a.n_tiles < 256 ? a.n_tiles : 256);
+    void* kargs[] = {&a, &f};
+    e = hipLaunchKernel(fn, dim3(grid), dim3(64 * S::WAVES), kargs, lds, (hipStream_t)stream);
+    if (e != hipSuccess) return (int)e;
+    return ZK_LAUNCH_CHECK();
+  }
+}
+
+}
diff --git a/zuko_amd/csrc/zk_ar_common.h b/zuko_amd/csrc/zk_ar_common.h
--- a/zuko_amd/csrc/zk_ar_common.h
+++ b/zuko_amd/csrc/zk_ar_common.h
@@ -60,6 +60,17 @@
   const float* base_scale;
 };
 
+struct ArhFlow {
+  int T;
+  int bias_stride;
+  int n_fmaps;
+  int term;
+  const float* bias;
+  const int32_t* featmap;
+  const float* table;
+};
+typedef int (*arhf_launch_fn)(const ArArgs* a, const ArhFlow* f, int abi, int args_bytes, int flow_bytes, void* stream);
+
 __device__ __forceinline__ float act_f32(float v, int act) {
   switch (act) {
     case 1: return v < 0.f ? 0.f : v;
diff --git a/zuko_amd/flows/autoregressive.py b/zuko_amd/flows/autoregressive.py
--- a/zuko_amd/flows/autoregressive.py
+++ b/zuko_amd/flows/autoregressive.py
@@ -653,3 +653,40 @@
         ]
         base = UnconditionalDistribution(DiagNormal, loc=torch.zeros(features), scale=torch.ones(features), buffer=True)
         super().__init__(layers, base)
+
+
+def fused_flow_call(transforms, x: Tensor, base=None):
+    if len(transforms) < 2 or not fused.fused_flow_enabled() or not torch.is_tensor(x) or x.dim() < 1:
+        return None
+    if any(type(t) is not FusedAutoregressiveTransform or t.c is not None for t in transforms):
+        return None
+    states = []
+    for t in transforms:
+        st = t._fused(x)
+        if st is None or not isinstance(st, fused.FusedAR):
+            return None
+        states.append(st)
+    flow = fused.flow_state(states, x.numel() // max(x.shape[-1], 1))
+    if flow is None:
+        return None
+    for t, st in zip(transforms, states):
+        t._check_widths(x, st)
+        st.refresh([m for m in t.lazy.hyper if isinstance(m, MaskedLinear)])
+    D = transforms[0].lazy.features
+    term = None
+    if base is not None and states[-1].serves_terminal() and all(v.dtype == torch.float32 and v.device == x.device and tuple(v.shape) == (D,) for v in base):
+        term = (base[0].contiguous(), base[1].contiguous())
+    if not flow.serves(term is not None):
+        return None
+    flow.sync()
+    batch = x.shape[:-1]
+    x2 = x.reshape(-1, D)
+    if not (x2.stride(-1) == 1 and x2.stride(0) % 4 == 0 and x2.data_ptr() % 16 == 0):
+        x2 = x2.contiguous()
+    ladj = torch.empty(x2.shape[0], dtype=x.dtype, device=x.device)
+    if term is not None:
+        flow.run(x2, None, ladj, base=term)
+        return None, ladj.reshape(batch)
+    y = torch.empty((x2.shape[0], D), dtype=x.dtype, device=x.device)
+    flow.run(x2, y, ladj)
+    return y.reshape(batch + (D,)), ladj.reshape(batch)
diff --git a/zuko_amd/fused.py b/zuko_amd/fused.py
--- a/zuko_amd/fused.py
+++ b/zuko_amd/fused.py
@@ -427,6 +427,104 @@
 HALF, GSPLIT, STATIC, GENERIC = range(4)
 
 
+def fused_flow_enabled() -> bool:
+    return os.environ.get("ZUKO_AMD_NO_FUSED_FLOW", "0") != "1"
+
+
+class FusedFlow:
+
+    def __init__(self, states: list, kernel, alt: list) -> None:
+        st0 = states[0]
+        self.states = list(states)
+        self.T = len(states)
+        self.kernel = kernel
+        self.per = st0.half_stream.buf.numel()
+        self.bias_stride = -(-st0.bias_floats // 256) * 256
+        dev = st0.device
+        self.stream = torch.zeros(self.T * self.per, dtype=torch.float32, device=dev)
+        self.bias = torch.zeros(self.T * self.bias_stride, dtype=torch.float32, device=dev)
+        maps, self.map_of = [], []
+        for st in states:
+            fm = np.asarray(st.plan.featmap, dtype=np.int32)
+            k = next((i for i, m in enumerate(maps) if np.array_equal(m, fm)), None)
+            if k is None:
+                maps.append(fm)
+                k = len(maps) - 1
+            self.map_of.append(k)
+        self.n_maps = len(maps)
+        self.featmap = torch.from_numpy(np.concatenate(maps)).to(dev)
+        self.table_host = np.zeros((self.T, 8), dtype=np.float32)
+        self.table_host.view(np.int32)[:, 4] = self.map_of
+        self.table_host.view(np.int32)[:, 5] = alt
+        self.table = torch.zeros(self.T * 8, dtype=torch.float32, device=dev)
+        self.stamps = [None] * self.T
+
+    @staticmethod
+    def build(states: list, rows):
+        from . import static_ar
+
+        st0 = states[0]
+        if len(states) < 2 or len(states) > 64 or any(st.half is None or st.half_stream is None or st.plan.fine_gather is None for st in states):
+            return None
+        if any(st.bias_floats != st0.bias_floats or st.act != st0.act or st.bound != st0.bound or st.slope != st0.slope or st.plan.layout.kind != st0.plan.layout.kind for st in states):
+            return None
+        tabs = [static_ar.half_tables(st.plan, st.plan.layout.kind, st.act) for st in states]
+        tf = None if any(t is None for t in tabs) else static_ar.flow_tables([t[0] for t in tabs])
+        if tf is None:
+            return None
+        p = st0.plan
+        n_maps = len({np.asarray(st.plan.featmap, dtype=np.int32).tobytes() for st in states})
+        stride = -(-st0.bias_floats // 256) * 256
+        xs = ((p.features + 3) // 4) * 4 + 4
+        if n_maps * len(p.featmap) > 1024 or (4 * tf[0]["CH"] * 256 + 2 * stride + 1024 + 256 + 8 * 16 * xs) * 4 > 160 * 1024:
+            return None
+        kernel = static_ar.lookup_flow(tf[0], rows)
+        return None if kernel is None else FusedFlow(states, kernel, tf[1])
+
+    def serves(self, terminal: bool) -> bool:
+        p = self.states[0].plan
+        if terminal and self.n_maps * len(p.featmap) + 3 * p.features > 1024:
+            return False
+        return all(st._half_serves(None) for st in self.states)
+
+    def sync(self) -> None:
+        dirty = False
+        for t, st in enumerate(self.states):
+            stamp = st.half_stream.stamp
+            if stamp != self.stamps[t]:
+                self.stream[t * self.per : (t + 1) * self.per].copy_(st.half_stream.buf)
+                self.bias[t * self.bias_stride : t * self.bias_stride + st.bias_floats].copy_(st.bias)
+                d = list(st.half_descale) + [1.0] * (4 - len(st.half_descale))
+                self.table_host[t, :4] = d
+                self.stamps[t] = stamp
+                dirty = True
+        if dirty:
+            self.table.copy_(torch.from_numpy(self.table_host.reshape(-1)))
+
+    def run(self, x: Tensor, y: Tensor | None, ladj: Tensor, base=None) -> None:
+        from . import _C
+        from .ops import _ptr, _stream
+
+        st0 = self.states[0]
+        p = st0.plan
+        io = dict(base_loc=_ptr(base[0]), base_scale=_ptr(base[1])) if base is not None else dict(y=_ptr(y), ldy=y.stride(0))
+        a = _C.args("zk_ar_args_v1", uni_kind=p.layout.kind, D=p.features, DIN=p.features, flow_transforms=self.T, n_layers=p.n_layers, n_groups=p.n_groups, n_chunks=st0.half_stream.n_chunks, act=st0.act,
+                    bias_floats=st0.bias_floats, flow_bias_stride=self.bias_stride, flow_featmaps=self.n_maps, N=x.shape[0], ldx=x.stride(0), bound=st0.bound, slope=st0.slope, x=_ptr(x), ladj=_ptr(ladj),
+                    wstream=_ptr(self.stream), bias=_ptr(self.bias), featmap=_ptr(self.featmap), flow_table=_ptr(self.table), launcher=self.kernel.launcher, **io)
+        _C.check(_C.lib().zk_ar_forward_static(a, _stream()), "zk_ar_forward_static (flow launch)")
+
+
+def flow_state(states: list, rows: int):
+    from . import static_ar
+
+    cache = states[0].__dict__.setdefault("_flows", {})
+    key = tuple((id(st), id(st.half)) for st in states)
+    jit = static_ar._jit_allowed(rows)
+    if key not in cache or (cache[key][0] is None and jit and not cache[key][1]):
+        cache[key] = (FusedFlow.build(states, rows), jit)
+    return cache[key][0]
+
+
 class FusedAR:
 
     def __init__(self, plan: ArPlan, device: torch.device, act: int, bound: float, slope: float, variant: int = 0) -> None:
diff --git a/zuko_amd/static_ar.py b/zuko_amd/static_ar.py
--- a/zuko_amd/static_ar.py
+++ b/zuko_amd/static_ar.py
@@ -325,6 +325,31 @@
     return out, g
 
 
+def flow_tables(tables: list):
+    t0 = tables[0]
+    if t0["NR"] != 4 or not t0["XLDS"] or t0["DIN"] != t0["D"] or t0["D"] % 4 or t0["NCHUNK"] < 2 or t0["STREAM_IMAGES"] != t0["NCHUNK"] * t0["CH"] or t0["BASE"][0] != 0:
+        return None
+    nb0 = t0["NB"][0]
+    alt, flags = None, []
+    for t in tables:
+        if t == t0:
+            flags.append(0)
+            continue
+        if {k: v for k, v in t.items() if k != "B_IP"} != {k: v for k, v in t0.items() if k != "B_IP"} or t["B_IP"][nb0:] != t0["B_IP"][nb0:] or (alt is not None and t["B_IP"][:nb0] != alt):
+            return None
+        alt = t["B_IP"][:nb0]
+        flags.append(1)
+    out = dict(t0, flow=1, FLOW_ALT=int(alt is not None), B_IP_ALT=alt if alt is not None else t0["B_IP"][:nb0])
+    return out, flags
+
+
+def lookup_flow(tf: dict, rows: int | None = None):
+    if not _enabled() or not half_enabled():
+        return None
+    found = find_or_compile(ARHF, tf, _jit_allowed(rows), verbose=_jit_verbose())
+    return None if found is None else found[0]
+
+
 HALF_LOOK = 1
 HALF_BPOS = 8
 
@@ -336,9 +361,25 @@
 
 
 def half_schedule(t: dict) -> tuple:
+    return _half_prologue(t), _half_pass(t)
+
+
+def _half_prologue(t: dict) -> list:
+    return [("issue",)] * (t["NR"] - 1) + [("x", t["NIT"]), ("wait", 0, True), ("barrier",)]
+
+
+def half_flow_bias_chunk(t: dict) -> int:
+    return t["NCHUNK"] - 2
+
+
+def half_flow_schedule(t: dict, T: int) -> tuple:
+    assert t["NR"] == 4 and t["NCHUNK"] >= 2
+    return _half_prologue(t), [_half_pass(t, rows=(k == T - 1), bias_at=half_flow_bias_chunk(t)) for k in range(T)]
+
+
+def _half_pass(t: dict, rows: bool = True, bias_at: int | None = None) -> list:
     ch, nr, per, look = t["CH"], t["NR"], t["CH"] // t["WAVES"], HALF_LOOK
     nit, last_base, images = t["NIT"], t["LAST_BASE"], t["IMAGES"]
-    pro = [("issue",)] * (nr - 1) + [("x", nit), ("wait", 0, True), ("barrier",)]
     if nr == 4:
         trig = {half_trigger(t, c): c for c in range(t["NCHUNK"])}
         xpos = min((p for p in trig if p >= last_base), default=-1)
@@ -348,10 +389,12 @@
 
     def read(pos):
         if nr != 4 and pos % ch == 0:
-            ev.extend([("wait", (nr - 2) * per + (nit if pos == xpos else 0), True), ("barrier",), ("issue",)])
+            ev.extend([("wait", (nr - 2) * per + (nit if pos == xpos and rows else 0), True), ("barrier",), ("issue",)])
         ev.append(("read", pos))
         if nr == 4 and pos in trig:
-            ev.extend([("wait", nit if pos == xpos else 0, pos % ch != t["BPOS"] + 1), ("barrier",), ("issue",)])
+            ev.extend([("wait", nit if pos == xpos and rows else 0, pos % ch != t["BPOS"] + 1), ("barrier",), ("issue",)])
+            if trig[pos] == bias_at:
+                ev.append(("bias",))
 
     def layer(base, nb, last_of):
         lk = min(look, nb)
@@ -369,12 +412,13 @@
         ots = t["B_OT"][off : off + nb]
         layer(t["BASE"][l], nb, lambda s: s + 1 == nb or ots[s + 1] != ots[s])
         off += nb
-    ev.append(("x", nit))
+    if rows:
+        ev.append(("x", nit))
     nbl = (images - last_base) // 2
     nt = nbl // max(t["GOFF"][-1], 1)
     ends = {g1 * nt - 1 for g1 in t["GOFF"][1:]}
     layer(last_base, nbl, lambda s: s in ends)
-    return pro, ev
+    return ev
 
 
 
@@ -415,6 +459,7 @@
     meta: object
 
 
+FLOW_ENTRY = "zk_arhf_launch"
 _FORWARD = dict(entry="zk_ars_launch", params=(("const zk::ArArgs*", "a"), ("int", "abi"), ("int", "args_bytes"), ("int", "train"), ("void*", "stream")))
 _BACKWARD = dict(entry="zk_ars_dgrad_launch", params=(("const zk::ArArgs*", "a"), ("int", "abi"), ("int", "args_bytes"), ("void*", "stream")))
 
@@ -443,6 +488,14 @@
     index=lambda t: "h" + _digest(t),
     meta=lambda t: dict(_pick(t, "uni", "ACT", "D", "DIN", "HT", "WAVES", "CH", "TRAIN_OK", "XLDS", "NCHUNK"), half=1, split=2),
 )
+ARHF = dataclasses.replace(
+    ARH, prefix="arhf", entry=FLOW_ENTRY, launcher="zk::arhf_launch<Shape, {uni}>",
+    params=(("const zk::ArArgs*", "a"), ("const zk::ArhFlow*", "f"), ("int", "abi"), ("int", "args_bytes"), ("int", "flow_bytes"), ("void*", "stream")),
+    shape=ARH.shape + (("bool", ("FLOW_ALT",)), ("unsigned char[]", ("B_IP_ALT",))),
+    sig=lambda t, alt: {"flow": t},
+    index=lambda t: "f" + _digest(t),
+    meta=lambda t: dict(_pick(t, "uni", "ACT", "D", "DIN", "HT", "WAVES", "CH", "XLDS", "NCHUNK", "NR", "FLOW_ALT"), half=1, flow=1),
+)
 ARSD_F32 = Family(
     prefix="arsd", header="fused_ar_static_impl.h", stamp=_header_digest, **_BACKWARD, launcher="zk::ars_dgrad_launch<Shape>",
     shape=(("int", ("DIN", "DOUT", "NIT", "NH", "TMAX", "NCHUNK", "WAVES=8", "ACT=1")), ("bool", ("HAS_ALT=false",)), ("int[]", ("HT", "NS", "BASE")),
@@ -460,7 +513,7 @@
 )
 ARSD_FULL = dataclasses.replace(
     ARSD_SPLIT, launcher="zk::arxb_launch<Shape, {uni}>", shape=ARSD_SPLIT.shape + (("int", ("NG",)), ("int[]", ("PB",))))
-FAMILIES = {"ars": ARS, "arx": ARX, "arh": ARH, "arsd": {1: ARSD_F32, 2: ARSD_SPLIT, 3: ARSD_FULL}}
+FAMILIES = {"ars": ARS, "arx": ARX, "arh": ARH, "arhf": ARHF, "arsd": {1: ARSD_F32, 2: ARSD_SPLIT, 3: ARSD_FULL}}
 
 
 def emit(fam: Family, t: dict, alt: list | None = None) -> str:
@@ -896,6 +949,10 @@
             th = half_tables(pl, layout.kind, act)
             if th is not None:
                 want(ARH, th[0])
+        tha, thd = (half_tables(pl, layout.kind, act) if pl is not None else None for pl in (pa, pd))
+        tf = flow_tables([tha[0], thd[0]]) if tha is not None and thd is not None else None
+        if tf is not None:
+            want(ARHF, tf[0])
         if layout.kind in SPLIT_ONLY_KINDS:
             continue
         ta, td = tables(pa, layout.kind, act), tables(pd, layout.kind, act)
diff --git a/zuko_amd/transforms.py b/zuko_amd/transforms.py
--- a/zuko_amd/transforms.py
+++ b/zuko_amd/transforms.py
@@ -409,6 +409,12 @@
 
     def call_and_ladj(self, x, base=None):
         dim = self.domain_dim
+        if dim == 1 and torch.is_tensor(x) and x.is_cuda and len(self.transforms) > 1:
+            from .flows.autoregressive import fused_flow_call
+
+            out = fused_flow_call(self.transforms, x, base)
+            if out is not None:
+                return out
         total = None
         owned = False
         last = self.transforms[-1]
```

Result: faster. 79.49 million samples/s (median of 6 runs) (+1.2%).
